# VGLoic/kzg-poly-commit-exploration

Measured on AMD Instinct MI355X. Metric: g1_msm_commitments_per_sec_degree_2^20, higher is better.
Workload: dtype i32 digits (Fp: 13 signed radix-2^30 digits, Montgomery 2^390; Fr: 8 x u32, Montgomery 2^256)

## Files before the change

### kzg_poly_commit_exploration_amd/csrc/api.hip

```cpp
#include <hip/hip_runtime.h>
#include <sys/random.h>

#include <algorithm>
#include <atomic>
#include <cerrno>
#include <chrono>
#include <condition_variable>
#include <cstdio>
#include <cstdlib>
#include <cstring>
#include <deque>
#include <functional>
#include <mutex>
#include <new>
#include <string>
#include <thread>
#include <vector>

#include "../../include/kzg_mi355x.h"
#include "engine.h"
#include "host_field.hpp"
#include "host_fr.hpp"
#include "fr30_host.hpp"
#include "host_pairing.hpp"
// ... 149 lines not shown
    DevBuf lag_part;
    DevBuf gp_in, gp_z, gp_part;
    PinnedBuf gp_flags{PinnedBuf::Mapped};
    DevBuf cpoly, cagg;
    SlotKind kind = SLOT_IDLE;
    size_t job_n = 0;
    uint32_t job_batch = 1;
    uint32_t open_y[8] = {};
    bool timing = false;
    bool has_quotient = false;
    bool tail_checked = false;
    kzg_kernel_times times = {};
};

}

struct kzg_ctx {
    kzg::MultiState* multi = nullptr;
    int device = 0;
    std::mutex mu;
    std::condition_variable slot_cv;
    int sync_owned = 0;
    bool raw_partials = false;
    bool host_trace = false;
    std::atomic<uint64_t> trace_ns[5] = {};
    std::atomic<uint64_t> trace_calls{0};
    std::string last_error;
    size_t n = 0;
    MsmConfig cfg = {};
    DevBuf table;
    DevBuf ntt_tw;
    DevBuf lag_table;
    size_t lag_n = 0;
    uint64_t srs_gen = 0;
    ReducePlan plan;
    size_t arena_records = 0, final_records = 0;
    uint32_t max_batch = 1;
    Slot slots[kNumSlots];
    hipStream_t front_stream = nullptr, heavy_stream = nullptr, tail_stream = nullptr;
    hipStream_t upload_stream = nullptr;
    uint32_t accum_lds_bytes = 41u * 1024u;
    uint32_t small_lds_bytes = 48u * 1024u;
    bool small_msm_off = false;
    bool slots_ready = false;
    bool timing = false;
    std::mutex fk20_mu;
    DevBuf glv;
    uint32_t glv_log = 0;
    DevBuf fk20_B, fk20_tab;
    uint32_t fk20_log_L = 0, fk20_log_l = 0;
    Workspace<11> fk20_ws;
    std::mutex recover_mu;
    DevBuf rec_g;
    Workspace<11> rec_ws;
    Workspace<17> vc_ws;
    Workspace<8> blob_ws;
    std::mutex lookup_mu;
    Workspace<6> lu_ws;
    std::mutex quotient_mu;
    Workspace<11> pq_ws;
    uint32_t pq_zinv_key = ~0u;
};

namespace {

#define HIP_TRY(ctx, expr)                                                                          \
    do {                                                                                            \
        hipError_t _e = (expr);                                                                     \
        if (_e != hipSuccess) {                                                                     \
            (ctx)->last_error = std::string(#expr) + ": " + hipGetErrorString(_e);                  \
            return KZG_ERR_HIP;                                                                     \
        }                                                                                           \
    } while (0)

int hip_fail(kzg_ctx* ctx, const char* what, hipError_t e) {
    ctx->last_error = std::string(what) + ": " + hipGetErrorString(e);
    return KZG_ERR_HIP;
}

struct TmpStream {
    hipStream_t s = nullptr;
    ~TmpStream() { if (s) hipStreamDestroy(s); }
};

int sync_unlocked(kzg_ctx* ctx, std::unique_lock<std::mutex>& lk, hipStream_t st, const char* what) {
    lk.unlock();
    const hipError_t e = hipStreamSynchronize(st);
    lk.lock();
    return e == hipSuccess ? KZG_OK : hip_fail(ctx, what, e);
}
constexpr const char* kCopyCoeffs = "hipMemcpyAsync (coefficients)";
int copy_unlocked(kzg_ctx* ctx, std::unique_lock<std::mutex>& lk, hipStream_t st, void* dst, const void* src, size_t bytes,
                  hipMemcpyKind kind, const char* what) {
    if (!bytes) return KZG_OK;
    lk.unlock();
    const hipError_t e = hipMemcpyAsync(dst, src, bytes, kind, st);
    lk.lock();
    return e == hipSuccess ? KZG_OK : hip_fail(ctx, what, e);
}

void free_slot_msm(Slot& s) {
    for (DevBuf* b : {&s.cnt, &s.offs, &s.block_sums, &s.pairs, &s.sorted, &s.buckets, &s.part_a, &s.part_b, &s.pair_scratch,
                      &s.heavy_ws, &s.arena})
        b->reset();
    s.fin.reset();
}

int create_stream(kzg_ctx* ctx, hipStream_t* out, bool high) {
    int least = 0, greatest = 0;
    HIP_TRY(ctx, hipDeviceGetStreamPriorityRange(&least, &greatest));
    const char* v = std::getenv("KZG_STREAM_PRIORITIES");
    const bool prio = !(v && v[0] == '0');
    HIP_TRY(ctx, hipStreamCreateWithPriority(out, hipStreamNonBlocking, prio ? (high ? greatest : least) : 0));
    return KZG_OK;
}

int ensure_slot_basics(kzg_ctx* ctx, Slot& s) {
    if (s.stream) return KZG_OK;
    if (!ctx->front_stream) {
        int rc = create_stream(ctx, &ctx->front_stream, false);
        if (rc) return rc;
    }
    if (!ctx->upload_stream) HIP_TRY(ctx, hipStreamCreateWithFlags(&ctx->upload_stream, hipStreamNonBlocking));
    for (auto& e : s.ev)
        if (!e) HIP_TRY(ctx, hipEventCreate(&e));
    if (!s.upload_ev) HIP_TRY(ctx, hipEventCreateWithFlags(&s.upload_ev, hipEventDisableTiming));
    s.stream = s.end = ctx->front_stream;
    if (!s.done) HIP_TRY(ctx, hipEventCreateWithFlags(&s.done, hipEventDisableTiming));
    return s.small.reserve(ctx, 64 * 4);
}

int upload_unlocked(kzg_ctx* ctx, std::unique_lock<std::mutex>& lk, Slot& s, void* dst, const void* src, size_t bytes) {
    if (!bytes) return KZG_OK;
    int rc = copy_unlocked(ctx, lk, ctx->upload_stream, dst, src, bytes, hipMemcpyHostToDevice, kCopyCoeffs);
    if (rc) return rc;
    HIP_TRY(ctx, hipEventRecord(s.upload_ev, ctx->upload_stream));
    HIP_TRY(ctx, hipStreamWaitEvent(s.stream, s.upload_ev, 0));
    return KZG_OK;
}

int ensure_poly(kzg_ctx* ctx, Slot& s, size_t n) {
    const size_t cap = n < 1024 ? 1024 : n;
    if (cap * 32 <= s.stage.cap) return KZG_OK;
    if (s.done) HIP_TRY(ctx, hipEventSynchronize(s.done));
    HIP_TRY(ctx, hipStreamSynchronize(ctx->upload_stream));
    HIP_TRY(ctx, hipStreamSynchronize(s.stream));
    for (DevBuf* b : {&s.stage, &s.q, &s.chunk, &s.block}) b->reset();
    int rc = s.stage.reserve(ctx, cap * 32);
    if (rc == KZG_OK) rc = s.q.reserve(ctx, cap * 32);
    if (rc == KZG_OK) rc = s.chunk.reserve(ctx, poly_chunk_words((uint32_t)cap) * 4);
    if (rc == KZG_OK) rc = s.block.reserve(ctx, poly_block_words((uint32_t)cap) * 4);
    if (rc) s.stage.reset();
    return rc;
}

void plan_reduce(kzg_ctx* ctx) {
    ReducePlan P;
    uint32_t bits = 0;
    while ((1u << bits) < ctx->cfg.nb) bits++;
    P.lo_bits = bits / 2;
    P.hi_bits = bits - P.lo_bits;
    P.row_lo = P.hi_bits / 2;
    P.row_hi = P.hi_bits - P.row_lo;
    P.col_lo = P.lo_bits / 2;
    P.col_hi = P.lo_bits - P.col_lo;
    P.off_r2row = 0;
    P.off_c2row = P.off_r2row + (1u << P.row_hi);
    P.off_r2col = P.off_c2row + (1u << P.row_lo);
    P.off_c2col = P.off_r2col + (1u << P.col_hi);
    P.total = P.off_c2col + (1u << P.col_lo);
    ctx->plan = P;
    ctx->arena_records = ((size_t)1 << P.hi_bits) + ((size_t)1 << P.lo_bits);
    ctx->final_records = P.total;
}

int setup_slots_impl(kzg_ctx* ctx);
int setup_slots(kzg_ctx* ctx, bool keep_table_on_failure = false) {
    ctx->slots_ready = false;
    int rc = setup_slots_impl(ctx);
    if (rc != KZG_OK) {
        for (auto& s : ctx->slots) free_slot_msm(s);
        if (keep_table_on_failure) return rc;
        ctx->table.reset();
        ctx->lag_table.reset();
        ctx->lag_n = 0;
        ctx->n = 0;
        (void)hipGetLastError();
    }
    return rc;
}
int setup_slots_impl(kzg_ctx* ctx) {
    plan_reduce(ctx);
    if (const char* v = std::getenv("KZG_TEST_FAIL_SLOT_ALLOC")) {
        const int mode = std::atoi(v);
        if (mode == 1 || (mode == 2 && ctx->max_batch > 1)) {
            ctx->last_error = "injected allocation failure (KZG_TEST_FAIL_SLOT_ALLOC)";
            return KZG_ERR_HIP;
        }
    }
    if (!ctx->heavy_stream) {
        int rc = create_stream(ctx, &ctx->heavy_stream, true);
        if (rc) return rc;
    }
    if (!ctx->tail_stream) {
        int rc = create_stream(ctx, &ctx->tail_stream, false);
        if (rc) return rc;
    }
    const MsmConfig cfg = ctx->cfg;
    if (ctx->max_batch > sort_max_batch(cfg)) ctx->max_batch = sort_max_batch(cfg);
    const size_t B = ctx->max_batch;
    const size_t pairs = (size_t)cfg.max_digits * ctx->n * B;
    for (int i = 0; i < kNumSlots; i++) {
        Slot& s = ctx->slots[i];
        {
            int rcb = ensure_slot_basics(ctx, s);
            if (rcb) return rcb;
        }
        if (!s.sorted_ev) {
            HIP_TRY(ctx, hipEventCreateWithFlags(&s.sorted_ev, hipEventDisableTiming));
            HIP_TRY(ctx, hipEventCreateWithFlags(&s.accum_ev, hipEventDisableTiming));
        }
        free_slot_msm(s);
        int rc = s.cnt.reserve(ctx, (size_t)sort_count_entries((uint32_t)B, cfg) * 4 + 64);
        if (rc == KZG_OK) rc = s.offs.reserve(ctx, ((size_t)cfg.nb * B + 1) * 4);
        if (rc == KZG_OK) rc = s.block_sums.reserve(ctx, (size_t)sort_workspace_words() * 4);
        if (rc) return rc;
        HIP_TRY(ctx, hipMemset(s.block_sums.p, 0, (size_t)sort_workspace_zero_words() * 4));
        rc = s.pairs.reserve(ctx, (pairs ? pairs : 1) * 8);
        if (rc == KZG_OK) rc = s.sorted.reserve(ctx, (pairs ? pairs : 1) * 4);
        if (rc == KZG_OK) rc = s.buckets.reserve(ctx, (size_t)cfg.nb * B * kXyzzBytes);
        if (rc == KZG_OK) rc = s.part_a.reserve(ctx, (size_t)kMaxAccumLanes * kXyzzBytes);
        if (rc == KZG_OK) rc = s.part_b.reserve(ctx, (size_t)kMaxAccumLanes * kXyzzBytes);
        if (rc == KZG_OK) rc = s.pair_scratch.reserve(ctx, accumulate_pair_scratch_bytes(pairs));
        if (rc == KZG_OK) rc = s.heavy_ws.reserve(ctx, heavy_workspace_bytes());
        if (rc == KZG_OK) rc = s.arena.reserve(ctx, ctx->arena_records * B * kXyzzBytes);
        if (rc == KZG_OK) rc = s.fin.reserve(ctx, ctx->final_records * B * kXyzzBytes);
        if (rc) return rc;
        s.kind = SLOT_IDLE;
    }
    ctx->slots_ready = true;
    return KZG_OK;
}

int build_tables(kzg_ctx* ctx, hipStream_t st, void* d_xyzz_tmp, void* d_prefix) {
    const size_t n = ctx->n;
    for (uint32_t j = 1; j < ctx->cfg.W; j++) {
        char* prev = (char*)ctx->table.p + (size_t)(j - 1) * n * kAffineBytes;
        char* next = (char*)ctx->table.p + (size_t)j * n * kAffineBytes;
        launch_table_window(st, prev, (uint32_t)n, ctx->cfg.level_bits, d_xyzz_tmp, d_prefix, next);
    }
    HIP_TRY(ctx, hipGetLastError());
    HIP_TRY(ctx, hipStreamSynchronize(st));
    return KZG_OK;
}

int drain_all(kzg_ctx* ctx) {
    for (hipStream_t st : {ctx->upload_stream, ctx->front_stream, ctx->heavy_stream, ctx->tail_stream})
        if (st) HIP_TRY(ctx, hipStreamSynchronize(st));
    return KZG_OK;
}

static int srs_release(kzg_ctx* ctx) {
    ctx->slots_ready = false;
    int rc = drain_all(ctx);
    if (rc) return rc;
    for (auto& s : ctx->slots) s.kind = SLOT_IDLE;
    ctx->table.reset();
    ctx->fk20_B.reset();
    ctx->fk20_tab.reset();
    ctx->lag_table.reset();
    ctx->lag_n = 0;
    ctx->srs_gen++;
    ctx->n = 0;
    return KZG_OK;
}

int srs_prepare(kzg_ctx* ctx, size_t n) {
    if (n == 0 || n > 0x7fffffffu / 32) return KZG_ERR_INVALID_ARG;
    int rc = srs_release(ctx);
    if (rc) return rc;
    size_t free_b = 0, total_b = 0;
    HIP_TRY(ctx, hipMemGetInfo(&free_b, &total_b));
    size_t budget = (size_t)((double)free_b * 0.6);
    if (const char* v = std::getenv("KZG_TABLE_GB")) budget = (size_t)(std::strtod(v, nullptr) * 1073741824.0);
    MsmConfig cfg = choose_msm_config(n, budget);
    if ((size_t)cfg.W * n >= 0x80000000ull) return KZG_ERR_INVALID_ARG;
    ctx->cfg = cfg;
    return ctx->table.reserve(ctx, (size_t)cfg.W * n * kAffineBytes);
}

struct MsmBasis {
    const void* table;
    uint32_t stride;
};
int enqueue_msm(kzg_ctx* ctx, Slot& s, const uint32_t* d_scalars, int is_mont, size_t n, int ev_base,
                uint32_t batch = 1, uint64_t stride = 0, const MsmBasis* basis = nullptr) {
    const MsmConfig cfg = ctx->cfg;
    const void* table = basis ? basis->table : ctx->table.p;
    const uint32_t table_stride = basis ? basis->stride : (uint32_t)ctx->n;
    const uint32_t nbt = cfg.nb * batch;
    hipStream_t st = s.stream;
    s.end = st;
    if (s.timing) HIP_TRY(ctx, hipEventRecord(s.ev[ev_base], st));
    const bool header_zeroed = launch_bucket_sort(st, d_scalars, is_mont, (uint32_t)n, batch, stride, table_stride, cfg, s.cnt.dev(),
                       s.block_sums.dev(), s.pairs.dev<uint64_t>(), s.offs.dev(), s.sorted.dev(), (uint32_t*)s.heavy_ws.p);
    if (s.timing) {
        HIP_TRY(ctx, hipEventRecord(s.ev[ev_base + 1], st));
        HIP_TRY(ctx, hipEventRecord(s.ev[ev_base + 2], st));
    }
    bool alone = true;
    for (const auto& other : ctx->slots) alone = alone && (&other == &s || other.kind == SLOT_IDLE);
    const uint64_t max_refs = (uint64_t)n * cfg.max_digits * batch;
    const uint32_t lanes = accumulate_lanes(max_refs, alone);
    const ReducePlan& P = ctx->plan;
    const uint32_t R = 1u << P.hi_bits, C = 1u << P.lo_bits, B = batch;
    char* row = (char*)s.arena.p;
    char* col = row + (size_t)R * B * kXyzzBytes;
    char* fin = (char*)s.fin.d;
    const uint32_t rl = 1u << P.row_lo, rh = 1u << P.row_hi, cl = 1u << P.col_lo, ch = 1u << P.col_hi;
    const TreeSumDesc stage1[2] = {
        {s.buckets.p, row, B * R, C, C, 1, B * R, 0},
        {s.buckets.p, col, B * C, R, 1, C, C, (uint64_t)cfg.nb}};
    const TreeSumDesc stage2[4] = {
        {row, fin + (size_t)P.off_r2row * B * kXyzzBytes, B * rh, rl, rl, 1, rh, R},
        {row, fin + (size_t)P.off_c2row * B * kXyzzBytes, B * rl, rh, 1, rl, rl, R},
        {col, fin + (size_t)P.off_r2col * B * kXyzzBytes, B * ch, cl, cl, 1, ch, C},
        {col, fin + (size_t)P.off_c2col * B * kXyzzBytes, B * cl, ch, 1, cl, cl, C}};
    if (!header_zeroed) HIP_TRY(ctx, hipMemsetAsync(s.heavy_ws.p, 0, kHeavyHeaderBytes, st));
    if (max_refs <= kTinyRefs && !ctx->small_msm_off) {
        if (s.timing) HIP_TRY(ctx, hipEventRecord(s.ev[ev_base + 3], st));
        launch_small_msm(st, table, s.sorted.dev(), s.offs.dev(), nbt, lanes, max_refs, s.buckets.p, s.part_a.p, s.part_b.p,
                         s.heavy_ws.p, s.small.dev() + 26, stage1, stage2, ctx->small_lds_bytes);
        if (s.timing) HIP_TRY(ctx, hipEventRecord(s.ev[ev_base + 4], st));
    } else {
        const bool hand_over = !alone;
        hipStream_t hs = hand_over ? ctx->heavy_stream : st;
        if (hand_over) {
            HIP_TRY(ctx, hipEventRecord(s.sorted_ev, st));
            HIP_TRY(ctx, hipStreamWaitEvent(hs, s.sorted_ev, 0));
        }
        if (s.timing) HIP_TRY(ctx, hipEventRecord(s.ev[ev_base + 3], hs));
        launch_bucket_accumulate(hs, table, s.sorted.dev(), s.offs.dev(), nbt, lanes, s.buckets.p, s.part_a.p, s.part_b.p,
                                 ctx->accum_lds_bytes, s.pair_scratch.p, max_refs,
                                 (char*)s.heavy_ws.p + kAccumClockOffset);
        if (s.timing) HIP_TRY(ctx, hipEventRecord(s.ev[ev_base + 4], hs));
        if (hand_over) {
            HIP_TRY(ctx, hipEventRecord(s.accum_ev, hs));
            st = s.end = ctx->tail_stream;
            HIP_TRY(ctx, hipStreamWaitEvent(st, s.accum_ev, 0));
        }
        launch_bucket_finalize(st, s.offs.dev(), nbt, lanes, s.part_a.p, s.part_b.p, s.buckets.p, s.heavy_ws.p, s.small.dev() + 26,
                               finalize_group_size(nbt));
        launch_tree_sums_two_stage(st, stage1, 2, stage2, 4, (uint32_t*)s.heavy_ws.p + 64, alone);
    }
    if (s.timing) HIP_TRY(ctx, hipEventRecord(s.ev[ev_base + 5], st));
    HIP_TRY(ctx, hipGetLastError());
    return KZG_OK;
}

hf::PX host_wsum(const uint64_t* recs, uint32_t len) {
    hf::PX run = hf::px_inf(), acc = hf::px_inf();
    for (uint32_t v = len; v-- > 1;) {
        run = hf::px_add(run, hf::px_from_record(recs + (size_t)v * kXyzzWords64));
        acc = hf::px_add(acc, run);
    }
    return acc;
}
hf::PX host_shift(hf::PX p, uint32_t k) {
    for (uint32_t i = 0; i < k; i++) p = hf::px_double(p);
    return p;
}
hf::P1 finish_msm(const kzg_ctx* ctx, const Slot& s, uint32_t p = 0, uint32_t batch = 1) {
    const ReducePlan& P = ctx->plan;
    const uint64_t* f = s.fin.host<uint64_t>();
    auto at = [&](uint32_t off, uint32_t len) { return f + ((size_t)off * batch + (size_t)p * len) * kXyzzWords64; };
    const uint32_t rh = 1u << P.row_hi, rl = 1u << P.row_lo, ch = 1u << P.col_hi, cl = 1u << P.col_lo;
    hf::PX w_row = hf::px_add(host_shift(host_wsum(at(P.off_r2row, rh), rh), P.row_lo), host_wsum(at(P.off_c2row, rl), rl));
    hf::PX w_col = hf::px_add(host_shift(host_wsum(at(P.off_r2col, ch), ch), P.col_lo), host_wsum(at(P.off_c2col, cl), cl));
    hf::PX total = hf::px_add(host_shift(w_row, P.lo_bits), w_col);
    if (ctx->cfg.recode == kRecodeNaf) total = hf::px_double(total);
    const uint64_t* r2 = at(P.off_r2row, rh);
    for (uint32_t k = 0; k < rh; k++) total = hf::px_add(total, hf::px_from_record(r2 + (size_t)k * kXyzzWords64));
    return ctx->raw_partials ? hf::px_to_jacobian(total) : hf::px_normalize(total);
}

void write_p1(uint64_t out[18], const hf::P1& p) { std::memcpy(out, &p, sizeof p); }

void fill_device_times(Slot& s) {
    s.times.references = s.small.host()[26];
    const uint64_t not_start = (uint64_t)s.small.host()[28] | ((uint64_t)s.small.host()[29] << 32);
    const uint64_t end = (uint64_t)s.small.host()[30] | ((uint64_t)s.small.host()[31] << 32);
    if (not_start != 0 && end > ~not_start) s.times.accumulate_ms = (float)((double)(end - ~not_start) * 1e-5);
}
void fill_accumulate_times(Slot& s) {
    float ms = 0;
    (void)hipEventElapsedTime(&ms, s.ev[3], s.ev[4]);
    s.times.accumulate_events_ms = ms;
    if (s.times.accumulate_ms == 0) s.times.accumulate_ms = ms;
}

void slot_idle(kzg_ctx* ctx, Slot& s) {
    s.kind = SLOT_IDLE;
    ctx->slot_cv.notify_all();
}
int reserve_slot(kzg_ctx* ctx, std::unique_lock<std::mutex>& lk, bool block) {
    for (;;) {
        for (int i = 0; i < kNumSlots; i++)
            if (ctx->slots[i].kind == SLOT_IDLE) {
                ctx->slots[i].kind = SLOT_RESERVED;
                ctx->sync_owned++;
                return i;
            }
        if (!block || ctx->sync_owned == 0) return -1;
        ctx->slot_cv.wait(lk);
    }
}
void release_owned(kzg_ctx* ctx, int slot) {
    if (ctx->slots[slot].kind == SLOT_RESERVED) ctx->slots[slot].kind = SLOT_IDLE;
    ctx->sync_owned--;
    ctx->slot_cv.notify_all();
}
struct SlotLease {
    kzg_ctx* ctx;
    int slot;
    ~SlotLease() { if (slot >= 0) release_owned(ctx, slot); }
};
void quiesce(kzg_ctx* ctx, std::unique_lock<std::mutex>& lk) {
    while (ctx->sync_owned > 0) ctx->slot_cv.wait(lk);
}

bool host_tail_nonzero(const uint64_t* coeffs, size_t from, size_t n) {
    for (size_t i = from; i < n; i++)
        if (coeffs[4 * i] | coeffs[4 * i + 1] | coeffs[4 * i + 2] | coeffs[4 * i + 3]) return true;
    return false;
}

int points_weights(kzg_ctx* ctx, const uint64_t* zs, size_t k, uint64_t* ws ) {
    if (k < 1 || k > KZG_MAX_OPEN_POINTS) {
        ctx->last_error = "multiproof: k must be in [1, KZG_MAX_OPEN_POINTS]";
        return KZG_ERR_INVALID_ARG;
    }
    hf::Fr z[KZG_MAX_OPEN_POINTS], w[KZG_MAX_OPEN_POINTS];
    std::memcpy(z, zs, 32 * k);
    if (!hf::fr_point_weights(z, k, w)) {
        ctx->last_error = "multiproof: two of the points are equal";
        return KZG_ERR_INVALID_ARG;
    }
    std::memcpy(ws, w, 32 * k);
    return KZG_OK;
}
int ensure_points(kzg_ctx* ctx, Slot& s, size_t n, size_t k) {
    int rc = s.roots.reserve(ctx, KZG_MAX_OPEN_POINTS * points_root_bytes());
    if (rc == KZG_OK) rc = s.pvals.reserve(ctx, KZG_MAX_OPEN_POINTS * 32);
    if (rc == KZG_OK) rc = s.pblock.reserve(ctx, k * poly_block_words((uint32_t)(n ? n : 1)) * 4, s.stream);
    return rc;
}
const uint32_t* points_values(const Slot& s, size_t k) { return k == 1 ? s.small.host() + 8 : s.pvals.host(); }
int enqueue_points_scan(kzg_ctx* ctx, Slot& s, const uint32_t* d_coeffs, size_t n, const uint64_t* zs, const uint64_t* ws,
                        size_t k, size_t nq, bool want_q) {
    std::memset(s.small.host(), 0, 64 * 4);
    std::memset(s.pvals.host(), 0, 32 * k);
    if (n == 0) return KZG_OK;
    if (k == 1) {
        uint32_t zw[8];
        std::memcpy(zw, zs, 32);
        uint32_t* q = want_q && n > 1 ? s.q.dev() : nullptr;
        if (!launch_quotient_single(s.stream, d_coeffs, (uint32_t)n, zw, q, s.small.dev())) {
            PolyScratch sc{s.chunk.dev(), s.block.dev(), s.small.dev(), s.small.dev() + 8};
            launch_quotient(s.stream, d_coeffs, (uint32_t)n, zw, q, sc);
        }
    } else {
        points_fill_roots(s.roots.h, zs, ws, (uint32_t)k, (uint32_t)n);
        HIP_TRY(ctx, hipMemcpyAsync(s.roots.d, s.roots.h, k * points_root_bytes(), hipMemcpyHostToDevice, s.stream));
        launch_quotient_points(s.stream, d_coeffs, (uint32_t)n, s.roots.d, (uint32_t)k, want_q ? s.q.dev() : nullptr, (uint32_t)nq,
                               s.pblock.dev(), s.pvals.dev());
    }
    HIP_TRY(ctx, hipGetLastError());
    return KZG_OK;
}

}

__global__ void k_tail_nonzero(const uint32_t* __restrict__ c, uint64_t from, uint64_t n, uint32_t* __restrict__ flag) {
    uint64_t i = from + (uint64_t)blockIdx.x * blockDim.x + threadIdx.x;
    if (i >= n) return;
    const uint4* p = reinterpret_cast<const uint4*>(c) + 2 * i;
    uint4 a = p[0], b = p[1];
    if (a.x | a.y | a.z | a.w | b.x | b.y | b.z | b.w) *flag = 1u;
}

#define KZG_SINGLE_DEVICE_ONLY(ctx)                                                                        \
    do {                                                                                                     \
        if ((ctx) && (ctx)->multi) {                                                                         \
            (ctx)->last_error = "this entry point takes a single-device context (kzg_ctx_create)";           \
            return KZG_ERR_INVALID_ARG;                                                                      \
        }                                                                                                    \
    } while (0)

extern "C" {

const char* kzg_strerror(int status) {
    switch (status) {
        case KZG_OK: return "ok";
        case KZG_ERR_DEGREE_TOO_HIGH:
            return "Setup does not allow for commitment generation of the polynomial. The polynomial degree is too high.";
        case KZG_ERR_CONSTANT_POLY: return "Unable to divide a constant polynomial";
        case KZG_ERR_REMAINDER:
            return "[divide_by_root] Fail to divide the polynomial by a root, constant terms do not add up";
        case KZG_ERR_INVALID_ARG: return "invalid argument";
        case KZG_ERR_NO_DEVICE: return "no HIP device available (this library has no CPU path)";
        case KZG_ERR_HIP: return "HIP runtime error";
        case KZG_ERR_NO_SRS: return "no SRS loaded";
        case KZG_ERR_BUSY: return "slot busy";
        default: return "unknown status";
    }
}

const char* kzg_last_error(const kzg_ctx* ctx) {
    if (!ctx) return "";
    if (ctx->multi && ctx->last_error.empty()) return multi_last_error(ctx->multi);
    return ctx->last_error.c_str();
}

int kzg_ctx_create_multi_ex(const int* devices, int ndev, unsigned flags, kzg_ctx** out) {
    if (!out) return KZG_ERR_INVALID_ARG;
    *out = nullptr;
    if (!devices || ndev <= 0 || (flags & ~(unsigned)KZG_MULTI_REPLICATE_SRS)) return KZG_ERR_INVALID_ARG;
    kzg::MultiState* m = nullptr;
    std::string err;
    int rc = multi_create(devices, ndev, (flags & KZG_MULTI_REPLICATE_SRS) ? kMultiReplicate : kMultiRange, &m, err);
    if (rc != KZG_OK) return rc;
    kzg_ctx* ctx = new kzg_ctx();
    ctx->multi = m;
    ctx->device = devices[0];
    *out = ctx;
    return KZG_OK;
}
int kzg_ctx_create_multi(const int* devices, int ndev, kzg_ctx** out) { return kzg_ctx_create_multi_ex(devices, ndev, 0u, out); }
int kzg_abi_version(void) { return KZG_ABI_VERSION; }
int kzg_num_devices(const kzg_ctx* ctx) { return !ctx ? 0 : (ctx->multi ? multi_num_devices(ctx->multi) : 1); }
uint64_t kzg_rccl_exchanges(const kzg_ctx* ctx) { return (ctx && ctx->multi) ? multi_rccl_exchanges(ctx->multi) : 0; }

int kzg_ctx_create(int device, kzg_ctx** out) {
    if (!out) return KZG_ERR_INVALID_ARG;
    *out = nullptr;
    int count = 0;
    if (hipGetDeviceCount(&count) != hipSuccess || count <= 0) return KZG_ERR_NO_DEVICE;
    if (device < 0 || device >= count) return KZG_ERR_NO_DEVICE;
    if (hipSetDevice(device) != hipSuccess) return KZG_ERR_NO_DEVICE;
    kzg_ctx* ctx = new kzg_ctx();
    ctx->device = device;
    if (const char* v = std::getenv("KZG_ACCUM_LDS_KB")) ctx->accum_lds_bytes = (uint32_t)std::atoi(v) * 1024u;
    if (const char* v = std::getenv("KZG_SMALL_MSM")) ctx->small_msm_off = std::atoi(v) == 0;
    if (const char* v = std::getenv("KZG_HOST_TRACE")) ctx->host_trace = std::atoi(v) != 0;
    if (hipFuncSetAttribute(small_msm_kernel(), hipFuncAttributeMaxDynamicSharedMemorySize, (int)small_msm_lds_bytes()) == hipSuccess)
        ctx->small_lds_bytes = small_msm_lds_bytes();
    else
        (void)hipGetLastError();
    if (!poly_prepare_device() || !points_prepare_device() || !sets_prepare_device()) {
        delete ctx;
        return KZG_ERR_HIP;
    }
    *out = ctx;
    return KZG_OK;
}

void kzg_ctx_destroy(kzg_ctx* ctx) {
    if (!ctx) return;
    if (ctx->multi) {
        multi_destroy(ctx->multi);
        delete ctx;
        return;
    }
    hipSetDevice(ctx->device);
    if (ctx->host_trace && ctx->trace_calls.load()) {
        const double k = 1e-3 / (double)ctx->trace_calls.load();
        std::fprintf(stderr, "[kzg host trace] %llu kzg_commit calls, us per call: wait-for-slot %.1f upload %.1f submit %.1f device %.1f collect %.1f\n",
                     (unsigned long long)ctx->trace_calls.load(), k * ctx->trace_ns[0].load(), k * ctx->trace_ns[1].load(),
                     k * ctx->trace_ns[2].load(), k * ctx->trace_ns[3].load(), k * ctx->trace_ns[4].load());
    }
    for (hipStream_t st : {ctx->upload_stream, ctx->front_stream, ctx->heavy_stream, ctx->tail_stream})
        if (st) hipStreamSynchronize(st);
    for (hipStream_t st : {ctx->upload_stream, ctx->front_stream, ctx->heavy_stream, ctx->tail_stream})
        if (st) hipStreamDestroy(st);
    delete ctx;
}

size_t kzg_srs_len(const kzg_ctx* ctx) { return !ctx ? 0 : (ctx->multi ? multi_srs_len(ctx->multi) : ctx->n); }
int kzg_num_slots(const kzg_ctx*) { return kNumSlots; }

int kzg_msm_config(const kzg_ctx* ctx, int* digit_bits, int* table_levels, size_t* num_buckets, int* recoding) {
    if (ctx && ctx->multi)
        return kzg_msm_config(multi_kid(ctx->multi, 0), digit_bits, table_levels, num_buckets, recoding);
    if (!ctx || !ctx->n) return KZG_ERR_NO_SRS;
    if (digit_bits) *digit_bits = (int)ctx->cfg.c;
    if (table_levels) *table_levels = (int)ctx->cfg.W;
    if (num_buckets) *num_buckets = ctx->cfg.nb;
    if (recoding) *recoding = (int)ctx->cfg.recode;
    return KZG_OK;
}

int kzg_srs_load_g1(kzg_ctx* ctx, const void* first_g1, size_t stride, size_t n) {
    if (!ctx || !first_g1 || stride < 144) return KZG_ERR_INVALID_ARG;
    if (ctx->multi) {
        std::lock_guard<std::mutex> lkm(ctx->mu);
        ctx->last_error.clear();
        return n ? multi_srs_load(ctx->multi, first_g1, stride, n) : KZG_ERR_INVALID_ARG;
    }
    std::unique_lock<std::mutex> lk(ctx->mu);
    quiesce(ctx, lk);
    HIP_TRY(ctx, hipSetDevice(ctx->device));
    int rc = srs_prepare(ctx, n);
    if (rc) return rc;
    std::vector<uint64_t> packed(n * 18);
    for (size_t i = 0; i < n; i++) std::memcpy(&packed[i * 18], (const char*)first_g1 + i * stride, 144);
    DevBuf d_jac, d_prefix, d_xyzz;
    HIP_TRY(ctx, hipMalloc(&d_jac.p, n * 144));
    HIP_TRY(ctx, hipMalloc(&d_prefix.p, n * 64));
    HIP_TRY(ctx, hipMalloc(&d_xyzz.p, n * kXyzzBytes));
    TmpStream st;
    HIP_TRY(ctx, hipStreamCreateWithFlags(&st.s, hipStreamNonBlocking));
    HIP_TRY(ctx, hipMemcpyAsync(d_jac.p, packed.data(), n * 144, hipMemcpyHostToDevice, st.s));
    ctx->n = n;
    launch_jacobian_to_affine(st.s, d_jac.p, (uint32_t)n, ctx->table.p, d_prefix.p);
    rc = build_tables(ctx, st.s, d_xyzz.p, d_prefix.p);
    if (rc) {
        ctx->n = 0;
        return rc;
    }
    return setup_slots(ctx);
}

int kzg_srs_generate_g1(kzg_ctx* ctx, const uint8_t secret_be[32], uint64_t first, size_t n) {
    if (!ctx || !secret_be) return KZG_ERR_INVALID_ARG;
    if (ctx->multi) {
        std::lock_guard<std::mutex> lkm(ctx->mu);
        ctx->last_error.clear();
        return n ? multi_srs_generate(ctx->multi, secret_be, first, n) : KZG_ERR_INVALID_ARG;
    }
    std::unique_lock<std::mutex> lk(ctx->mu);
    quiesce(ctx, lk);
    HIP_TRY(ctx, hipSetDevice(ctx->device));
    int rc = srs_prepare(ctx, n);
    if (rc) return rc;
    uint32_t raw[8];
// ... 6351 lines not shown
```

### kzg_poly_commit_exploration_amd/csrc/engine.h

```cpp
#pragma once
#include <hip/hip_runtime.h>
#include <stddef.h>
#include <stdint.h>

namespace kzg {

constexpr size_t kAffineBytes = 128;
constexpr size_t kAffineU4 = kAffineBytes / 16;
constexpr size_t kXyzzBytes = 256;
constexpr size_t kXyzzU4 = kXyzzBytes / 16;
constexpr size_t kXyzzWords64 = kXyzzBytes / 8;

enum : uint32_t { kRecodeWindows = 0, kRecodeNaf = 1 };
struct MsmConfig {
    uint32_t recode;
    uint32_t c;
    uint32_t W;
    uint32_t level_bits;
    uint32_t nb;
    uint32_t max_digits;
};

MsmConfig choose_msm_config(size_t n_points, size_t table_budget_bytes);

constexpr uint32_t kTinyRefs = 65536;
__host__ __device__ inline uint32_t accumulate_min_seg(uint64_t refs) { return refs <= kTinyRefs ? 4u : 8u; }
__host__ __device__ inline uint32_t accumulate_seg_len(uint32_t M, uint32_t lanes) {
    uint32_t L = (M + lanes - 1) / lanes;
    const uint32_t lo = accumulate_min_seg(M);
    return L < lo ? lo : L;
}

constexpr size_t kHeavyHeaderBytes = 1024;
uint32_t sort_count_entries(uint32_t max_batch, MsmConfig cfg);
uint32_t sort_max_batch(MsmConfig cfg);
uint32_t sort_workspace_words();
uint32_t sort_workspace_zero_words();
bool launch_bucket_sort(hipStream_t s, const uint32_t* d_scalars, int scalars_are_mont, uint32_t n, uint32_t batch,
                        uint64_t stride, uint32_t table_stride, MsmConfig cfg, uint32_t* d_cnt,
                        uint32_t* d_ws, uint64_t* d_pairs, uint32_t* d_offs, uint32_t* d_sorted, uint32_t* d_header);
constexpr uint32_t kMaxAccumLanes = 262144 + 64;
uint32_t accumulate_lanes(uint64_t max_refs, bool alone = false);
size_t accumulate_pair_scratch_bytes(uint64_t max_refs);
void launch_bucket_accumulate(hipStream_t s, const void* d_table, const uint32_t* d_sorted, const uint32_t* d_offs,
                              uint32_t nb, uint32_t lanes, void* d_buckets ,
                              void* d_part_a, void* d_part_b, uint32_t lds_reserve_bytes, void* d_pair_scratch,
                              uint64_t max_refs, void* d_clock = nullptr );
constexpr size_t kAccumClockOffset = 768;
size_t heavy_workspace_bytes();
void launch_bucket_finalize(hipStream_t s, const uint32_t* d_offs, uint32_t nb, uint32_t lanes, const void* d_part_a,
                            const void* d_part_b, void* d_buckets, void* d_heavy_ws,
                            uint32_t* d_refs_out , uint32_t group = 1);
uint32_t finalize_group_size(uint32_t nb);
struct TreeSumDesc;
uint32_t small_msm_lds_bytes();
const void* small_msm_kernel();
void launch_small_msm(hipStream_t s, const void* d_table, const uint32_t* d_sorted, const uint32_t* d_offs, uint32_t nb,
                      uint32_t lanes, uint64_t max_refs, void* d_buckets, void* d_part_a, void* d_part_b, void* d_heavy_ws,
                      uint32_t* d_refs_out, const TreeSumDesc* stage1 , const TreeSumDesc* stage2 ,
                      uint32_t lds_bytes);
struct TreeSumDesc {
    const void* in;
    void* out;
    uint32_t groups, len;
    uint64_t gstride, estride;
    uint32_t inner;
    uint64_t ostride;
};
void launch_tree_sums(hipStream_t s, const TreeSumDesc* descs, uint32_t count, bool dense = false, bool alone = true);
void launch_tree_sums_two_stage(hipStream_t s, const TreeSumDesc* stage1, uint32_t count1, const TreeSumDesc* stage2,
                                uint32_t count2, uint32_t* d_sync, bool alone);

void launch_jacobian_to_affine(hipStream_t s, const void* d_jac, uint32_t n, void* d_affine_out,
                               void* d_prefix_tmp);
void launch_table_window(hipStream_t s, const void* d_prev_affine, uint32_t n, uint32_t c,
                         void* d_xyzz_tmp, void* d_prefix_tmp, void* d_next_affine);
void launch_srs_generate(hipStream_t s, const uint32_t* secret_raw8 , uint64_t first, uint32_t n,
                         void* d_gtable, void* d_xyzz_tmp, void* d_prefix_tmp, void* d_affine_out);
size_t srs_gtable_bytes();
void launch_affine96_to_table(hipStream_t s, const void* d_affine96, uint32_t n, void* d_table);
void launch_uncompress(hipStream_t s, const void* d_compressed, uint32_t n, void* d_table, uint32_t* d_status);

void launch_wire_g1(hipStream_t s, const void* d_in48, const uint32_t* d_src, uint32_t n, void* d_records, uint32_t stride_bytes,
                    uint32_t* d_err);
void launch_wire_fr(hipStream_t s, const void* d_in32, uint32_t n, uint32_t log_row, bool bit_reversed, void* d_out, uint32_t* d_err);

void launch_enc_g1(hipStream_t s, const void* d_affine, uint32_t n, uint32_t log_row, bool bit_reversed, void* d_out48);
void launch_enc_fr(hipStream_t s, const void* d_in, uint32_t n, uint32_t log_row, uint32_t log_cells, bool bit_reversed, void* d_out32,
                   uint32_t* d_err);
struct Fr30;
void launch_poly_trim(hipStream_t s, void* d_coeffs, uint32_t n, uint64_t stride, uint32_t batch, const Fr30* scale, uint32_t* d_out);

void launch_affine_to_p1(hipStream_t s, const void* d_affine, uint32_t n, void* d_p1_out);

struct Fr30;
constexpr uint32_t kNttMaxLog = 22;
constexpr uint32_t kNttTableLen = 2048;
constexpr uint32_t kNttTileLog = 11;
constexpr uint32_t kNttTile = 1u << kNttTileLog;
constexpr uint32_t kNttMaxRadixLog = 9;
struct NttPlan {
    uint32_t passes;
    uint32_t m[3];
};
NttPlan ntt_plan(uint32_t log_n);
bool ntt_prepare_device();
void launch_ntt(hipStream_t s, const uint32_t* d_in, uint32_t* d_out, uint32_t log_n, const void* d_tw, const Fr30& last_c,
                uint32_t* d_buf_a, uint32_t* d_buf_b);

uint32_t cells_chunk_log(uint32_t nq, uint32_t log_l);
uint64_t cells_agg_words(uint32_t nq, uint32_t log_l, uint32_t cells);
void launch_cell_quotients(hipStream_t s, const uint32_t* d_coeffs, uint32_t nq, uint32_t log_n, uint32_t log_l,
                           uint32_t first_cell, uint32_t cells, const void* d_tw, uint32_t* d_agg, uint32_t* d_q,
                           uint64_t stride);
void launch_cells_gather(hipStream_t s, const uint32_t* d_evals, uint32_t* d_out, uint32_t log_n, uint32_t log_l);

struct Glv {
    uint64_t k1[2], k2[2];
};
constexpr uint32_t kFk20CombWindows = 64;
constexpr uint32_t kFk20CombDigits = 8;
constexpr uint32_t kFk20CombEntries = kFk20CombWindows * kFk20CombDigits;
const void* launch_g1_dft(hipStream_t s, const void* d_in, void* d_a, void* d_b, uint32_t log_len, uint64_t batch,
                          const Glv* d_tw, uint32_t log_tw, bool inverse);
void launch_g1_scale(hipStream_t s, void* d_io, uint64_t n, const Glv& k);
void launch_fk20_srs_gather(hipStream_t s, const void* d_table, uint64_t srs_n, uint32_t log_L, uint32_t log_l, void* d_out);
void launch_fk20_comb(hipStream_t s, const void* d_bases, uint32_t log_L, uint32_t log_l, uint64_t first, uint32_t count,
                      void* d_tmp);
const uint32_t* launch_fk20_fr_side(hipStream_t s, const uint32_t* d_coeffs, uint32_t n, uint32_t m, uint32_t log_L,
                                    uint32_t log_l, uint64_t batch, const void* d_tw, const Fr30& inv_L, uint32_t* d_a,
                                    uint32_t* d_b);
void launch_fk20_pointwise(hipStream_t s, const uint32_t* d_scal, const void* d_tab, uint32_t log_L, uint32_t log_l,
                           uint32_t i0, uint32_t ci, uint64_t batch, void* d_part, void* d_out);
void launch_fk20_select(hipStream_t s, const void* d_conv, uint32_t log_L, uint32_t m, uint32_t log_M, uint64_t batch, void* d_H);
void launch_affine_to_xyzz(hipStream_t s, const void* d_affine, uint64_t n, void* d_out);
void launch_xyzz_to_affine(hipStream_t s, const void* d_xyzz, uint32_t n, void* d_out, void* d_prefix);
const uint32_t* launch_fr_dft(hipStream_t s, const uint32_t* d_in, uint32_t* d_a, uint32_t* d_b, uint32_t log_len, uint64_t batch,
                              const void* d_tw);

uint32_t recover_vanish_parts(uint32_t n_missing);
void launch_recover_vanishing(hipStream_t s, const uint32_t* d_missing, uint32_t n_missing, const void* d_tw, uint32_t log_n,
                              uint32_t log_l, const Fr30& gl, uint32_t* d_part, uint32_t* d_z);
void launch_recover_scatter(hipStream_t s, const uint32_t* d_cells, const int32_t* d_pos, const uint32_t* d_zrecv, uint32_t k,
                            uint32_t log_n, uint32_t log_l, uint64_t batch, uint32_t* d_out);
void launch_recover_twist(hipStream_t s, uint32_t* d_io, uint32_t log_n, uint64_t batch, const void* d_gtab, const Fr30& c);
void launch_recover_divide(hipStream_t s, uint32_t* d_io, uint32_t log_n, uint32_t log_l, uint64_t batch, const uint32_t* d_zinv);
void launch_recover_untwist(hipStream_t s, uint32_t* d_io, uint32_t log_n, uint32_t n, uint64_t batch, const void* d_ginv,
                            const Fr30& c, uint32_t* d_coef, bool pad, uint32_t* d_flags);
void launch_recover_gather(hipStream_t s, const uint32_t* d_in, uint32_t* d_out, uint32_t log_n, uint32_t log_l, uint64_t batch);

void launch_vc_ladder(hipStream_t s, const void* d_rec, const uint32_t* d_src, const Glv* d_glv, uint32_t lanes, uint32_t n_check,
                      uint32_t split, void* d_out_a, void* d_out_b, uint32_t* d_err);
void launch_vc_cell_scale(hipStream_t s, const void* d_T, const uint32_t* d_ids, uint32_t D, const Glv* d_tw, uint32_t shift,
                          void* d_out);
void launch_vc_g1_sum(hipStream_t s, const void* d_in, const uint32_t* d_starts, uint32_t groups, void* d_out);
void launch_vc_fr_sum(hipStream_t s, const uint32_t* d_in, const uint32_t* d_order, const Fr30* d_rho, const uint32_t* d_starts,
                      uint32_t groups, uint32_t log_l, uint32_t* d_out);
void launch_vc_fr_twist(hipStream_t s, uint32_t* d_io, const uint32_t* d_ids, uint32_t D, const void* d_itw, uint32_t log_n,
                        uint32_t log_l, const Fr30& inv_l);

void launch_srs_update(hipStream_t s, const uint32_t* tau_raw8, uint64_t first, uint32_t n, const void* d_level0, void* d_out_xyzz);
void launch_srs_check(hipStream_t s, const void* d_level0, uint32_t n, uint32_t* d_err);

constexpr uint32_t kBaryThreads = 256;
constexpr uint32_t kBaryRun = 4;
constexpr uint32_t kBaryTile = kBaryThreads * kBaryRun;
constexpr uint32_t kBaryPartialWords = 12;
inline uint32_t bary_tiles(uint32_t log_n) { return (uint32_t)((((uint64_t)1 << log_n) + kBaryTile - 1) / kBaryTile); }
void launch_bary(hipStream_t s, const uint32_t* d_evals, uint32_t log_n, uint32_t batch, const Fr30* d_zs, const void* d_tw,
                 const Fr30& inv_n, uint32_t* d_partial, uint32_t* d_out);

constexpr uint32_t kLagTile = 1024;
constexpr uint32_t kLagPartialWords = 24;
inline uint32_t lagrange_tiles(uint32_t log_n) { return (uint32_t)((((uint64_t)1 << log_n) + kLagTile - 1) / kLagTile); }
void launch_lagrange_quotient(hipStream_t s, const uint32_t* d_evals, uint32_t log_n, const Fr30& z, const Fr30& y, const Fr30& inv_n,
                              const void* d_tw, uint32_t* d_q, uint32_t* d_partial, uint32_t* d_flags);

constexpr uint32_t kGpTile = 1024;
constexpr uint32_t kGpCarryThreads = 256;
constexpr uint32_t kGpPartialWords = 24;
constexpr uint32_t kGpMaxColumns = 16;
constexpr uint32_t kGpNone = 0xffffffffu;
inline uint32_t gp_tiles(size_t n) { return (uint32_t)((n + kGpTile - 1) / kGpTile); }
struct GpOut {
    uint32_t* d_z;
    uint32_t* d_partial;
    uint32_t* d_flags;
};
void launch_grand_product(hipStream_t s, const uint32_t* d_nums, const uint32_t* d_dens, uint32_t n, uint32_t t, size_t stride,
                          const Fr30& scale, const Fr30& img_one, const GpOut& out);
void launch_permutation_product(hipStream_t s, const uint32_t* d_wires, const uint32_t* d_sigmas, uint32_t log_n, uint32_t t,
                                size_t stride, const Fr30* bk, const Fr30& beta, const Fr30& gamma, const void* d_tw,
                                const Fr30& scale, const Fr30& img_one, const GpOut& out);

constexpr uint32_t kLuTile = 512;
constexpr uint32_t kLuCarryThreads = 256;
constexpr uint32_t kLuMaxColumns = 16;
constexpr uint32_t kLuNone = 0xffffffffu;
constexpr uint32_t kLuRecD = 0, kLuRecHit = 9, kLuRecW = 10, kLuRecC = 20, kLuRecBase = 32, kLuPartialWords = 40;
inline uint32_t lu_tiles(size_t n) { return (uint32_t)((n + kLuTile - 1) / kLuTile); }
struct LuOut {
    uint32_t* d_phi;
    uint32_t* d_partial;
    uint32_t* d_flags;
};
void launch_logderivative_sum(hipStream_t s, const uint32_t* d_nums, const uint32_t* d_dens, uint32_t n, uint32_t t, size_t stride,
                              const Fr30& scale, const Fr30& img_one, const LuOut& out);
void launch_lookup_sum(hipStream_t s, const uint32_t* d_lookups, uint32_t n, uint32_t k, size_t stride, const uint32_t* d_table,
                       const uint32_t* d_mult, const Fr30& beta, const Fr30& scale, const Fr30& img_one, const LuOut& out);
void launch_batch_inverse(hipStream_t s, const uint32_t* d_vals, uint32_t n, const Fr30& scale, const Fr30& img_one, const LuOut& out);
struct LuHash {
    uint32_t* d_slots;
    uint32_t log_cap;
    uint32_t* d_counts;
    uint32_t* d_words;
};
void launch_lookup_multiplicities(hipStream_t s, const uint32_t* d_table, uint32_t n_table, const uint32_t* d_lookups, uint32_t n,
                                  uint32_t k, size_t stride, const LuHash& h, const Fr30& count_img, uint32_t* d_out_mult,
                                  uint32_t* d_out_rows, uint32_t* d_flags);

constexpr uint32_t kPqTile = 256;
constexpr uint32_t kPqMaxColumns = 7;
constexpr uint32_t kPqMaxLogExt = 3;
struct PqColumns {
    const uint32_t *d_wires, *d_sigmas, *d_z, *d_l0, *d_gate, *d_zinv;
};
struct PqScalars {
    const Fr30 *beta, *gamma, *one, *alpha1, *alpha2;
    const Fr30* bkg;
};
void launch_pq_constraints(hipStream_t s, const PqColumns& cols, uint32_t log_N, uint32_t rot, uint32_t t, size_t stride,
                           const PqScalars& sc, const void* d_tw, uint32_t* d_out);
void launch_pq_pad_twist(hipStream_t s, const uint32_t* d_in, size_t stride, uint32_t len, const Fr30& fill, uint32_t log_N,
                         uint64_t batch, const void* d_gtab, const Fr30& c, uint32_t* d_out);

constexpr uint32_t kCombineThreads = 256;
constexpr uint32_t kCombineTile = 2048;
constexpr uint32_t kCombinePartialWords = 12;
constexpr uint32_t kCombineMax = 256;
constexpr uint32_t kCombineTabPa = 0;
constexpr uint32_t kCombineTabPb = 16;
constexpr uint32_t kCombineTabZ256 = 32;
constexpr uint32_t kCombineTabWa = 33;
constexpr uint32_t kCombineTabWb = 49;
constexpr uint32_t kCombineTabW256 = 65;
constexpr uint32_t kCombineTabGamma = 66;
constexpr uint32_t kCombineTabLen = kCombineTabGamma + kCombineMax;
inline uint32_t combine_tiles(uint32_t n) { return (uint32_t)(((uint64_t)n + kCombineTile - 1) / kCombineTile); }
void launch_combine_eval(hipStream_t s, const uint32_t* d_coeffs, uint32_t n, uint32_t t, uint64_t stride, const Fr30* d_tab,
                         uint32_t first, bool carry, uint32_t* d_f, uint32_t* d_partial, uint32_t* d_ys);
constexpr uint32_t kSetsMax = 8;
constexpr uint32_t kSetsMaxPoints = 16;
constexpr uint32_t kSetsMaxValues = kCombineMax * kSetsMaxPoints;
void launch_sets_combine(hipStream_t s, const uint32_t* d_coeffs, uint32_t n, uint32_t t, uint64_t stride, const Fr30* d_tab,
                         const Fr30* d_mult, const uint32_t* d_sel, uint32_t sel_base, bool carry, uint32_t* d_g, uint32_t* d_partial,
                         uint32_t* d_ys);

}
#include <string>
struct kzg_ctx;
namespace kzg {
void ctx_set_raw_partials(kzg_ctx* ctx, bool raw);
int ctx_drop_srs(kzg_ctx* ctx);
int ctx_commit_batch_host(kzg_ctx* ctx, const uint64_t* coeffs, size_t n, size_t stride_coeffs, size_t first, size_t step,
                          size_t count, uint64_t* out_p1s);
int ctx_open_batch_host(kzg_ctx* ctx, const uint64_t* coeffs, size_t n, size_t stride_coeffs, size_t first, size_t step,
                        size_t count, const uint64_t* zs, const uint64_t* ys, uint64_t* out_p1s, int* statuses);
int ctx_open_slice_begin(kzg_ctx* ctx, const uint64_t* slice, size_t len, const uint64_t z[4], uint64_t out_h[4], int* slot_out);
int ctx_open_slice_finish(kzg_ctx* ctx, int slot, size_t len, const uint64_t carry[4], const uint64_t z[4],
                          const uint64_t start[4], uint64_t out_p1[18]);
void ctx_open_slice_abort(kzg_ctx* ctx, int slot);

struct MultiState;
enum : uint32_t { kMultiRange = 0, kMultiReplicate = 1 };
int multi_create(const int* devices, int ndev, uint32_t mode, MultiState** out, std::string& err);
void multi_destroy(MultiState* m);
size_t multi_srs_len(const MultiState* m);
int multi_num_devices(const MultiState* m);
uint64_t multi_rccl_exchanges(const MultiState* m);
kzg_ctx* multi_kid(MultiState* m, int g);
const char* multi_last_error(const MultiState* m);
int multi_srs_generate(MultiState* m, const uint8_t secret_be[32], uint64_t first, size_t n);
int multi_srs_load(MultiState* m, const void* first_g1, size_t stride, size_t n);
int multi_srs_load_affine(MultiState* m, const void* affine_xy, size_t n);
int multi_srs_load_compressed(MultiState* m, const uint8_t* compressed, size_t n, size_t* bad_index);
int multi_srs_read(MultiState* m, size_t index, size_t count, uint64_t* out_p1);
int multi_commit(MultiState* m, const void* scalars, int is_mont, size_t n, uint64_t out_p1[18]);
int multi_open(MultiState* m, const uint64_t* coeffs, size_t n, const uint64_t z[4], const uint64_t y[4], uint64_t out_p1[18]);
int multi_commit_batch(MultiState* m, const uint64_t* coeffs, size_t n, size_t batch, size_t stride_coeffs, uint64_t* out_p1s);
int multi_open_batch(MultiState* m, const uint64_t* coeffs, size_t n, size_t batch, size_t stride_coeffs, const uint64_t* zs,
                     const uint64_t* ys, uint64_t* out_p1s, int* statuses);
int multi_open_points(MultiState* m, const uint64_t* coeffs, size_t n, const uint64_t* zs, const uint64_t* ys, size_t k,
                      uint64_t out_p1[18]);
int multi_open_combined(MultiState* m, const uint64_t* coeffs, size_t n, size_t t, size_t stride, const uint64_t z[4],
                        const uint64_t gamma[4], uint64_t* out_ys, uint64_t out_p1[18]);
int multi_open_sets(MultiState* m, const uint64_t* coeffs, size_t n, size_t t, size_t stride, const uint32_t* set_of,
                    const uint32_t* set_len, size_t nsets, const uint64_t* zs, const uint64_t gamma[4], uint64_t* out_ys,
                    uint64_t out_p1[18]);
int multi_set_max_batch(MultiState* m, size_t max_batch);
uint32_t multi_mode(const MultiState* m);

struct PolyScratch {
    uint32_t* d_chunk;
    uint32_t* d_block;
    uint32_t* d_flags;
    uint32_t* d_result;
};
bool poly_prepare_device();
size_t poly_chunk_words(uint32_t n);
size_t poly_block_words(uint32_t n);
bool launch_quotient_single(hipStream_t s, const uint32_t* d_coeffs, uint32_t n, const uint32_t z_mont[8], uint32_t* d_q,
                            uint32_t* d_small);
void launch_quotient(hipStream_t s, const uint32_t* d_coeffs, uint32_t n, const uint32_t z_mont[8],
                     uint32_t* d_q, PolyScratch scratch);
bool points_prepare_device();
size_t points_root_bytes();
void points_fill_roots(void* h_roots, const uint64_t* zs_mont, const uint64_t* ws_mont, uint32_t k, uint32_t n);
void launch_quotient_points(hipStream_t s, const uint32_t* d_coeffs, uint32_t n, const void* d_roots, uint32_t k, uint32_t* d_q,
                            uint32_t nq, uint32_t* d_block, uint32_t* d_vals);
bool sets_prepare_device();
void launch_quotient_sets(hipStream_t s, const uint32_t* d_g, uint32_t n, const void* d_roots, uint32_t k, uint32_t* d_q,
                          uint32_t* d_block, uint32_t* d_vals);

constexpr uint32_t kBlobProofMaxN = 4096;
constexpr uint32_t kBlobProofZWords = 12;
bool launch_blobproof_quotients(hipStream_t s, const uint32_t* d_coeffs, uint32_t n, uint64_t stride, uint32_t batch,
                                const uint32_t* d_z, uint32_t* d_q, uint32_t* d_flags);

}
```

### kzg_poly_commit_exploration_amd/csrc/msm_accum.hip

```cpp
#include <cstdlib>

#ifndef KZG_ACCUM_PARALLEL_COLUMNS
#define KZG_F30_SERIAL_COLUMNS 1
#endif
#include "engine.h"
#include "field30_inv.hip.h"
#include "g1_30.hip.h"

namespace kzg {

#ifndef KZG_ACCUM_BLOCK
#define KZG_ACCUM_BLOCK 256
#endif
constexpr int kAccumBlock = KZG_ACCUM_BLOCK;

__device__ __forceinline__ Fq load_fq(const uint4* __restrict__ p) {
    const uint4 a = p[0], b = p[1], c = p[2];
    const uint32_t d = reinterpret_cast<const uint32_t*>(p)[12];
    Fq r;
    r.d[0] = (int32_t)a.x; r.d[1] = (int32_t)a.y; r.d[2] = (int32_t)a.z; r.d[3] = (int32_t)a.w;
    r.d[4] = (int32_t)b.x; r.d[5] = (int32_t)b.y; r.d[6] = (int32_t)b.z; r.d[7] = (int32_t)b.w;
    r.d[8] = (int32_t)c.x; r.d[9] = (int32_t)c.y; r.d[10] = (int32_t)c.z; r.d[11] = (int32_t)c.w;
    r.d[12] = (int32_t)d;
    return r;
}
__device__ __forceinline__ Affine30 load_affine30(const uint4* __restrict__ table, uint32_t idx) {
    const uint4* p = table + (size_t)idx * kAffineU4;
    Affine30 r;
    r.x = load_fq(p);
    r.y = load_fq(p + 4);
    return r;
}

__device__ __forceinline__ uint32_t bucket_of(const uint32_t* __restrict__ offs, uint32_t nb, uint32_t pos) {
    uint32_t lo = 0, hi = nb;
    while (hi - lo > 1) {
        uint32_t mid = (lo + hi) >> 1;
        if (offs[mid] <= pos) lo = mid; else hi = mid;
    }
    return lo;
}

typedef __attribute__((address_space(3))) char* lds_char_ptr;
typedef uint32_t accum_u32x4 __attribute__((ext_vector_type(4)));
typedef const __attribute__((address_space(3))) accum_u32x4* lds_u4_ptr;
extern __shared__ uint4 lds_points[];
__device__ __forceinline__ uint32_t accum_wave_lane() { return __builtin_amdgcn_mbcnt_hi(~0u, __builtin_amdgcn_mbcnt_lo(~0u, 0u)); }
__device__ __forceinline__ uint32_t accum_wave_slot() {
    const uint32_t lds0 = (uint32_t)(uintptr_t)(lds_char_ptr)(char*)lds_points;
    return lds0 + __builtin_amdgcn_readfirstlane(threadIdx.x >> 6) * (8u * 64u * 16u);
}
__device__ __forceinline__ void accum_issue_gather(const uint4* __restrict__ table, uint32_t slot, uint32_t r) {
    const char* src = reinterpret_cast<const char*>(table + (size_t)(r & 0x7fffffffu) * kAffineU4);
#pragma unroll
    for (int k = 0; k < 8; k++)
        __builtin_amdgcn_global_load_lds((const __attribute__((address_space(1))) void*)(src + 16 * k),
                                         (__attribute__((address_space(3))) void*)(lds_char_ptr)(uintptr_t)(slot + 1024u * k),
                                         16, 0, 0);
}
constexpr int kFlushOps = 17;
static_assert(kFlushOps == 17, "the literal in accum_take_point's s_waitcnt");
__device__ __forceinline__ Affine30 accum_read_point(uint32_t lane_slot) {
    Affine30 r;
    lds_u4_ptr q = (lds_u4_ptr)(uintptr_t)lane_slot;
    const accum_u32x4 x0 = q[0], x1 = q[64], x2 = q[128], x3 = q[192];
    const accum_u32x4 y0 = q[256], y1 = q[320], y2 = q[384], y3 = q[448];
    r.x.d[0] = (int32_t)x0.x; r.x.d[1] = (int32_t)x0.y; r.x.d[2] = (int32_t)x0.z; r.x.d[3] = (int32_t)x0.w;
    r.x.d[4] = (int32_t)x1.x; r.x.d[5] = (int32_t)x1.y; r.x.d[6] = (int32_t)x1.z; r.x.d[7] = (int32_t)x1.w;
    r.x.d[8] = (int32_t)x2.x; r.x.d[9] = (int32_t)x2.y; r.x.d[10] = (int32_t)x2.z; r.x.d[11] = (int32_t)x2.w;
    r.x.d[12] = (int32_t)x3.x;
    r.y.d[0] = (int32_t)y0.x; r.y.d[1] = (int32_t)y0.y; r.y.d[2] = (int32_t)y0.z; r.y.d[3] = (int32_t)y0.w;
    r.y.d[4] = (int32_t)y1.x; r.y.d[5] = (int32_t)y1.y; r.y.d[6] = (int32_t)y1.z; r.y.d[7] = (int32_t)y1.w;
    r.y.d[8] = (int32_t)y2.x; r.y.d[9] = (int32_t)y2.y; r.y.d[10] = (int32_t)y2.z; r.y.d[11] = (int32_t)y2.w;
    r.y.d[12] = (int32_t)y3.x;
    return r;
}
__device__ __forceinline__ Affine30 accum_take_point(uint32_t slot, bool wave_flushed = false) {
#ifdef KZG_ACCUM_FULL_WAIT
    wave_flushed = false;
#endif
    if (wave_flushed) asm volatile("s_waitcnt vmcnt(17)" ::: "memory");
    else asm volatile("s_waitcnt vmcnt(0)" ::: "memory");
    const Affine30 r = accum_read_point(slot + accum_wave_lane() * 16u);
    asm volatile("s_waitcnt lgkmcnt(0)" ::: "memory");
    return r;
}
struct AccumRare {
    XYZZ30 acc;
    Fq P, Rn;
};
static __device__ __noinline__ bool accum_rare_call(AccumRare* io) { return xyzz30_acc_rare(io->acc, io->P, io->Rn); }
__device__ __forceinline__ void accum_flush_run(uint4* dst, const XYZZ30& a) {
    const Fq* f[4] = {&a.X, &a.Y, &a.ZZ, &a.ZZZ};
    accum_u32x4 v[16];
#pragma unroll
    for (int c = 0; c < 4; c++) {
        v[4 * c + 0] = accum_u32x4{(uint32_t)f[c]->d[0], (uint32_t)f[c]->d[1], (uint32_t)f[c]->d[2], (uint32_t)f[c]->d[3]};
        v[4 * c + 1] = accum_u32x4{(uint32_t)f[c]->d[4], (uint32_t)f[c]->d[5], (uint32_t)f[c]->d[6], (uint32_t)f[c]->d[7]};
        v[4 * c + 2] = accum_u32x4{(uint32_t)f[c]->d[8], (uint32_t)f[c]->d[9], (uint32_t)f[c]->d[10], (uint32_t)f[c]->d[11]};
        v[4 * c + 3] = accum_u32x4{(uint32_t)f[c]->d[12], 0u, 0u, 0u};
    }
    asm volatile(
        "global_store_dwordx4 %0, %1, off\n\t"
        "global_store_dwordx4 %0, %2, off offset:16\n\t"
        "global_store_dwordx4 %0, %3, off offset:32\n\t"
        "global_store_dwordx4 %0, %4, off offset:48\n\t"
        "global_store_dwordx4 %0, %5, off offset:64\n\t"
        "global_store_dwordx4 %0, %6, off offset:80\n\t"
        "global_store_dwordx4 %0, %7, off offset:96\n\t"
        "global_store_dwordx4 %0, %8, off offset:112\n\t"
        "global_store_dwordx4 %0, %9, off offset:128\n\t"
        "global_store_dwordx4 %0, %10, off offset:144\n\t"
        "global_store_dwordx4 %0, %11, off offset:160\n\t"
        "global_store_dwordx4 %0, %12, off offset:176\n\t"
        "global_store_dwordx4 %0, %13, off offset:192\n\t"
        "global_store_dwordx4 %0, %14, off offset:208\n\t"
        "global_store_dwordx4 %0, %15, off offset:224\n\t"
        "global_store_dwordx4 %0, %16, off offset:240"
        :
        : "v"(dst), "v"(v[0]), "v"(v[1]), "v"(v[2]), "v"(v[3]), "v"(v[4]), "v"(v[5]), "v"(v[6]), "v"(v[7]), "v"(v[8]), "v"(v[9]),
          "v"(v[10]), "v"(v[11]), "v"(v[12]), "v"(v[13]), "v"(v[14]), "v"(v[15])
        : "memory");
}
__device__ __forceinline__ uint32_t accum_ref(const uint32_t* __restrict__ sorted, uint32_t i) {
    return *reinterpret_cast<const uint32_t*>(reinterpret_cast<const char*>(sorted) + (uint32_t)(i * 4u));
}

#ifndef KZG_ACCUM_MIN_BLOCKS
#define KZG_ACCUM_MIN_BLOCKS 2
#endif
__global__ void __launch_bounds__(kAccumBlock, KZG_ACCUM_MIN_BLOCKS)
k_bucket_accumulate(const uint4* __restrict__ table, const uint32_t* __restrict__ sorted, const uint32_t* __restrict__ offs,
                    uint32_t nb, uint32_t lanes, uint4* __restrict__ buckets, uint4* __restrict__ part_a,
                    uint4* __restrict__ part_b, unsigned long long* __restrict__ clk) {
    asm volatile("" ::: "v175");
    const bool stamp = clk != nullptr && (threadIdx.x & 63) == 0;
    if (stamp) atomicMax(&clk[0], ~(unsigned long long)wall_clock64());
    const uint32_t lane = blockIdx.x * kAccumBlock + threadIdx.x;
    const uint32_t M = offs[nb];
    const uint32_t L = accumulate_seg_len(M, lanes);
    const uint64_t start64 = (uint64_t)lane * L;
    if (start64 >= M) return;
    const uint32_t start = (uint32_t)start64;
    const uint32_t end = (M - start < L) ? M : start + L;

    uint32_t b = bucket_of(offs, nb, start);
    uint32_t b_beg = offs[b], b_end = offs[b + 1];
    uint32_t b_end_next = offs[(b + 2 <= nb) ? b + 2 : nb];
    uint32_t run_start = start;
    XYZZ30 acc = xyzz30_inf();
    const uint32_t wave_slot = accum_wave_slot();
    uint32_t ref = accum_ref(sorted, start);
    uint32_t ref_next = accum_ref(sorted, min(start + 1, M - 1));
    accum_issue_gather(table, wave_slot, ref);
    for (uint32_t e = start; e < end; e++) {
        const bool wave_flushed = __builtin_amdgcn_ballot_w64(e == b_end) != 0;
        if (e == b_end) {
            uint4* dst = (run_start == b_beg) ? buckets + (size_t)b * kXyzzU4 : part_a + (size_t)lane * kXyzzU4;
            xyzz30_acc_settle(acc);
            accum_flush_run(dst, acc);
            acc = xyzz30_inf();
            b++;
            b_beg = b_end;
            b_end = b_end_next;
            while (b_end <= e) {
                b++;
                b_beg = b_end;
                b_end = offs[b + 1];
            }
            b_end_next = offs[(b + 2 <= nb) ? b + 2 : nb];
            run_start = e;
        }
        Fq P, Rn;
        uint32_t code;
        {
            const Affine30 p = accum_take_point(wave_slot, wave_flushed);
            code = xyzz30_acc_head(acc, p, (ref >> 31) != 0, P, Rn);
        }
        bool more = code == 0;
        if (__builtin_amdgcn_ballot_w64(code != 0) != 0) {
            if (code & kAccFresh) {
                if (!(code & kAccPointInf)) {
                    const Affine30 p = accum_read_point(wave_slot + accum_wave_lane() * 16u);
                    xyzz30_acc_set(acc, p, (ref >> 31) != 0);
                }
            } else if (code == kAccMaybeEqual) {
                AccumRare t;
                t.acc = acc;
                t.P = P;
                t.Rn = Rn;
                more = accum_rare_call(&t);
                acc = t.acc;
                P = t.P;
                Rn = t.Rn;
                __builtin_amdgcn_s_waitcnt(0x0f70);
            }
        }
        ref = ref_next;
        if (e + 1 < end) accum_issue_gather(table, wave_slot, ref);
        ref_next = accum_ref(sorted, min(e + 2, M - 1));
        if (more) xyzz30_acc_tail(acc, P, Rn);
    }
    uint4* dst;
    if (run_start == b_beg && end == b_end) dst = buckets + (size_t)b * kXyzzU4;
    else if (run_start == start) dst = part_a + (size_t)lane * kXyzzU4;
    else dst = part_b + (size_t)lane * kXyzzU4;
    xyzz30_acc_settle(acc);
    store_xyzz30(dst, acc);
    if (stamp) atomicMax(&clk[1], (unsigned long long)wall_clock64());
}

constexpr uint32_t kPairRecU4 = 4;

static __device__ __noinline__ Fq fq_mul_call(Fq a, Fq b) { return fq_mul(a, b); }
static __device__ __noinline__ Fq fq_sqr_call(Fq a) { return fq_sqr(a); }
#ifdef KZG_PAIR_CALLS
#define KZG_PAIR_MUL(a, b) fq_mul_call(a, b)
#define KZG_PAIR_SQR(a) fq_sqr_call(a)
#else
#define KZG_PAIR_MUL(a, b) fq_mul(a, b)
#define KZG_PAIR_SQR(a) fq_sqr(a)
#endif
static __device__ __noinline__ void fq_inv_call(Fq* io) {
    const Fq a = *io;
    *io = fq_inv(a);
}
static __device__ __noinline__ uint32_t pair_classify_call(const Affine30* a, bool nega, const Affine30* b, bool negb, Fq* den) {
    Fq d;
    const uint32_t kind = pair_classify(*a, nega, *b, negb, d);
    *den = d;
    return kind;
}

__global__ void __launch_bounds__(kAccumBlock, 2) k_bucket_accumulate_pairs(const uint4* __restrict__ table,
                                                                            const uint32_t* __restrict__ sorted,
                                                                            const uint32_t* __restrict__ offs, uint32_t nb,
                                                                            uint32_t lanes, uint4* __restrict__ buckets,
                                                                            uint4* __restrict__ part_a,
                                                                            uint4* __restrict__ part_b,
                                                                            uint4* __restrict__ prefix_buf) {
    const uint32_t lane = blockIdx.x * kAccumBlock + threadIdx.x;
    const uint32_t M = offs[nb];
    const uint32_t L = accumulate_seg_len(M, lanes);
    const uint64_t start64 = (uint64_t)lane * L;
    if (start64 >= M) return;
    const uint32_t start = (uint32_t)start64;
    const uint32_t end = (M - start < L) ? M : start + L;
    const uint32_t J = (end - start + 1) / 2;
    auto rec = [&](uint32_t j, uint32_t piece) { return prefix_buf + ((size_t)(j * kPairRecU4 + piece) * lanes + lane); };
    uint4* const slot0 = lds_points + (threadIdx.x >> 6) * (16 * 64);
    uint4* const slot1 = slot0 + 8 * 64;
    const uint32_t wl = threadIdx.x & 63;
    auto dma = [&](uint4* slot, uint32_t r, int first_piece, int pieces) {
        const char* src = reinterpret_cast<const char*>(table + (size_t)(r & 0x7fffffffu) * kAffineU4);
#pragma unroll
        for (int k = 0; k < 8; k++)
            if (k >= first_piece && k < first_piece + pieces)
                __builtin_amdgcn_global_load_lds((const __attribute__((address_space(1))) void*)(src + 16 * k),
                                                 (__attribute__((address_space(3))) void*)(slot + 64 * k), 16, 0, 0);
    };
    auto lds_fq = [&](const uint4* slot, int first_piece) {
        const uint4 a = slot[64 * first_piece + wl], b2 = slot[64 * (first_piece + 1) + wl], c = slot[64 * (first_piece + 2) + wl],
                    d = slot[64 * (first_piece + 3) + wl];
        Fq r;
        r.d[0] = (int32_t)a.x; r.d[1] = (int32_t)a.y; r.d[2] = (int32_t)a.z; r.d[3] = (int32_t)a.w;
        r.d[4] = (int32_t)b2.x; r.d[5] = (int32_t)b2.y; r.d[6] = (int32_t)b2.z; r.d[7] = (int32_t)b2.w;
        r.d[8] = (int32_t)c.x; r.d[9] = (int32_t)c.y; r.d[10] = (int32_t)c.z; r.d[11] = (int32_t)c.w;
        r.d[12] = (int32_t)d.x;
        return r;
    };

    uint32_t b = bucket_of(offs, nb, start);
    uint32_t b_end = offs[b + 1];
    Fq run = fq_one();
    {
        uint32_t r0 = sorted[start], r1 = start + 1 < end ? sorted[start + 1] : 0u;
        uint32_t r0n = start + 2 < end ? sorted[start + 2] : 0u, r1n = start + 3 < end ? sorted[start + 3] : 0u;
        dma(slot0, r0, 0, 4);
        dma(slot1, r1, 0, 4);
        for (uint32_t j = 0; j < J; j++) {
            const uint32_t e0 = start + 2 * j, e1 = e0 + 1;
            while (b_end <= e0) {
                b++;
                b_end = offs[b + 1];
            }
            asm volatile("s_waitcnt vmcnt(0)" ::: "memory");
            const Fq x0 = lds_fq(slot0, 0), x1 = lds_fq(slot1, 0);
            asm volatile("s_waitcnt lgkmcnt(0)" ::: "memory");
            const uint32_t c0 = r0, c1 = r1;
            if (j + 1 < J) {
                r0 = r0n;
                r1 = r1n;
                dma(slot0, r0, 0, 4);
                dma(slot1, r1, 0, 4);
                r0n = e0 + 4 < end ? sorted[e0 + 4] : 0u;
                r1n = e0 + 5 < end ? sorted[e0 + 5] : 0u;
            }
            uint32_t kind = kPairNone;
            Fq den = fq_one();
            if (e1 < end && e1 < b_end) {
                const Fq dx = fq_norm(fq_sub_raw(x1, x0));
                if (!fq_all_zero(x0) && !fq_all_zero(x1) && !fq_is_zero(dx)) {
                    kind = kPairAdd;
                    den = dx;
                } else {
                    Affine30 a, c;
                    a.x = x0;
                    a.y = load_fq(table + (size_t)(c0 & 0x7fffffffu) * kAffineU4 + 4);
                    c.x = x1;
                    c.y = load_fq(table + (size_t)(c1 & 0x7fffffffu) * kAffineU4 + 4);
                    kind = pair_classify_call(&a, (c0 >> 31) != 0, &c, (c1 >> 31) != 0, &den);
                }
            }
            *rec(j, 0) = make_uint4((uint32_t)run.d[0], (uint32_t)run.d[1], (uint32_t)run.d[2], (uint32_t)run.d[3]);
            *rec(j, 1) = make_uint4((uint32_t)run.d[4], (uint32_t)run.d[5], (uint32_t)run.d[6], (uint32_t)run.d[7]);
            *rec(j, 2) = make_uint4((uint32_t)run.d[8], (uint32_t)run.d[9], (uint32_t)run.d[10], (uint32_t)run.d[11]);
            *rec(j, 3) = make_uint4((uint32_t)run.d[12], kind, c0, c1);
            if (kind == kPairAdd || kind == kPairDouble) run = KZG_PAIR_MUL(run, den);
        }
    }
    Fq inv = run;
    fq_inv_call(&inv);

    b = bucket_of(offs, nb, end - 1);
    uint32_t b_beg = offs[b];
    b_end = offs[b + 1];
    XYZZ30 acc = xyzz30_inf();
    auto flush = [&]() {
        uint4* dst;
        if (b_beg >= start && b_end <= end) dst = buckets + (size_t)b * kXyzzU4;
        else if (b_beg <= start) dst = part_a + (size_t)lane * kXyzzU4;
        else dst = part_b + (size_t)lane * kXyzzU4;
        store_xyzz30(dst, acc);
    };
    auto enter = [&](uint32_t e) {
        if (e < b_beg) {
            flush();
            acc = xyzz30_inf();
            do {
                b--;
                b_end = b_beg;
                b_beg = offs[b];
            } while (b_beg > e);
        }
    };
    uint32_t e = end - 1;
    auto ref_at = [&](uint32_t idx_plus_1) { return idx_plus_1 > start ? sorted[idx_plus_1 - 1] : 0u; };
    uint32_t w0 = sorted[e], w1 = ref_at(e), w2 = e >= 1 ? ref_at(e - 1) : 0u, w3 = e >= 2 ? ref_at(e - 2) : 0u;
    uint4 q0, q1, q2, q3;
    {
        const uint32_t j = (e - start) >> 1;
        q0 = *rec(j, 0); q1 = *rec(j, 1); q2 = *rec(j, 2); q3 = *rec(j, 3);
        dma(slot1, w0, 0, 8);
        dma(slot0, w1, 0, 8);
    }
    bool more_steps = true;
    while (more_steps) {
        asm volatile("s_waitcnt vmcnt(0)" ::: "memory");
        const uint32_t j = (e - start) >> 1;
        const uint32_t kind = q3.y;
        const bool second = ((e - start) & 1u) != 0;
        const bool paired = kind != kPairNone && second;
        const uint32_t r_hi = w0, r_lo = w1;
        Fq prefix;
        prefix.d[0] = (int32_t)q0.x; prefix.d[1] = (int32_t)q0.y; prefix.d[2] = (int32_t)q0.z; prefix.d[3] = (int32_t)q0.w;
        prefix.d[4] = (int32_t)q1.x; prefix.d[5] = (int32_t)q1.y; prefix.d[6] = (int32_t)q1.z; prefix.d[7] = (int32_t)q1.w;
        prefix.d[8] = (int32_t)q2.x; prefix.d[9] = (int32_t)q2.y; prefix.d[10] = (int32_t)q2.z; prefix.d[11] = (int32_t)q2.w;
        prefix.d[12] = (int32_t)q3.x;
        Affine30 pt;
        pt.x = lds_fq(slot1, 0);
        pt.y = lds_fq(slot1, 4);
        Affine30 lo;
        lo.x = lds_fq(slot0, 0);
        lo.y = lds_fq(slot0, 4);
        asm volatile("s_waitcnt lgkmcnt(0)" ::: "memory");
        enter(e);
        const uint32_t used = paired ? 2u : 1u;
        more_steps = e >= start + used;
        if (more_steps) {
            e -= used;
            if (paired) { w0 = w2; w1 = w3; } else { w0 = w1; w1 = w2; w2 = w3; }
            const uint32_t jn = (e - start) >> 1;
            q0 = *rec(jn, 0); q1 = *rec(jn, 1); q2 = *rec(jn, 2); q3 = *rec(jn, 3);
            dma(slot1, w0, 0, 8);
            dma(slot0, w1, 0, 8);
            if (paired) {
                w2 = e >= start + 2 ? sorted[e - 2] : 0u;
                w3 = e >= start + 3 ? sorted[e - 3] : 0u;
            } else {
                w3 = e >= start + 3 ? sorted[e - 3] : 0u;
            }
        }
        bool neg = (r_hi >> 31) != 0;
        bool have = true;
        if (paired) {
            const bool n0 = (r_lo >> 31) != 0;
            if (kind == kPairCancel) {
                have = false;
            } else if (kind == kPairOnlyA) {
                pt = lo;
                neg = n0;
            } else if (kind != kPairOnlyB) {
                const Fq den = kind == kPairAdd ? fq_norm(fq_sub_raw(pt.x, lo.x)) : fq_norm(fq_add_raw(fq_cneg(lo.y, n0), fq_cneg(pt.y, neg)));
                const Fq inv_den = KZG_PAIR_MUL(inv, prefix);
                KZG_SB30();
                inv = KZG_PAIR_MUL(inv, den);
                KZG_SB30();
                pt = pair_sum_with(kind, lo, n0, pt, neg, inv_den, [](const Fq& x, const Fq& y) { return KZG_PAIR_MUL(x, y); },
                                   [](const Fq& x) { return KZG_PAIR_SQR(x); });
                neg = false;
            }
        }
        if (have) xyzz30_madd(acc, pt, neg);
    }
    flush();
}

__global__ void __launch_bounds__(64) k_fq_table_to_p1(const uint4* __restrict__ table, uint32_t n, uint4* __restrict__ out) {
    const uint32_t i = blockIdx.x * 64 + threadIdx.x;
    if (i >= n) return;
    const Affine30 a = load_affine30(table, i);
    uint32_t w[36];
#pragma unroll
    for (int t = 0; t < 36; t++) w[t] = 0;
    if (!(fq_all_zero(a.x) && fq_all_zero(a.y))) {
        fq_to_u32x12(a.x, w);
        fq_to_u32x12(a.y, w + 12);
        constexpr uint32_t ONE[12] = {0x0002fffdu, 0x76090000u, 0xc40c0002u, 0xebf4000bu, 0x53c758bau, 0x5f489857u,
                                      0x70525745u, 0x77ce5853u, 0xa256ec6du, 0x5c071a97u, 0xfa80e493u, 0x15f65ec3u};
#pragma unroll
        for (int t = 0; t < 12; t++) w[24 + t] = ONE[t];
    }
    uint4* o = out + (size_t)i * 9;
#pragma unroll
    for (int t = 0; t < 9; t++) o[t] = make_uint4(w[4 * t], w[4 * t + 1], w[4 * t + 2], w[4 * t + 3]);
}
void launch_affine_to_p1(hipStream_t s, const void* d_affine, uint32_t n, void* d_p1) {
    if (!n) return;
    hipLaunchKernelGGL(k_fq_table_to_p1, dim3((n + 63) / 64), dim3(64), 0, s, (const uint4*)d_affine, n, (uint4*)d_p1);
}

uint32_t accumulate_lanes(uint64_t max_refs, bool alone) {
    (void)alone;
    static const uint64_t target = [] {
        const char* v = std::getenv("KZG_ACCUM_LANES");
        uint64_t l = v ? std::strtoull(v, nullptr, 10) : 131072ull;
        return l < 64 ? 131072ull : (l > 262144ull ? 262144ull : l);
    }();
    const uint64_t lo = accumulate_min_seg(max_refs);
    uint64_t lanes = (max_refs + lo - 1) / lo;
    if (lanes > target) lanes = target;
    lanes = (lanes + kAccumBlock - 1) / kAccumBlock * kAccumBlock;
    return (uint32_t)lanes;
}

bool accumulate_pairs_enabled() {
    static const int pairs_mode = [] {
        const char* v = std::getenv("KZG_ACCUM_PAIRS");
        return v ? std::atoi(v) : 0;
    }();
    return pairs_mode != 0;
}
size_t accumulate_pair_scratch_bytes(uint64_t max_refs) {
    if (!accumulate_pairs_enabled()) return 0;
    return (size_t)(max_refs / 2 + kMaxAccumLanes) * kPairRecU4 * 16;
}

void launch_bucket_accumulate(hipStream_t s, const void* d_table, const uint32_t* d_sorted, const uint32_t* d_offs,
                              uint32_t nb, uint32_t lanes, void* d_buckets, void* d_part_a, void* d_part_b,
                              uint32_t lds_reserve_bytes, void* d_pair_scratch, uint64_t max_refs, void* d_clock) {
    if (!lanes) return;
    if (accumulate_pairs_enabled() && d_pair_scratch && max_refs / lanes >= 16) {
        hipLaunchKernelGGL(k_bucket_accumulate_pairs, dim3(lanes / kAccumBlock), dim3(kAccumBlock),
                           (kAccumBlock / 64) * 16 * 64 * 16 , s,
                           reinterpret_cast<const uint4*>(d_table), d_sorted, d_offs, nb, lanes,
                           reinterpret_cast<uint4*>(d_buckets), reinterpret_cast<uint4*>(d_part_a),
                           reinterpret_cast<uint4*>(d_part_b), reinterpret_cast<uint4*>(d_pair_scratch));
        return;
    }
    const uint32_t need = (kAccumBlock / 64) * 8 * 64 * 16;
    lds_reserve_bytes = lds_reserve_bytes / (256 / kAccumBlock);
    if (lds_reserve_bytes < need) lds_reserve_bytes = need;
    hipLaunchKernelGGL(k_bucket_accumulate, dim3(lanes / kAccumBlock), dim3(kAccumBlock), lds_reserve_bytes, s,
                       reinterpret_cast<const uint4*>(d_table), d_sorted, d_offs, nb, lanes,
                       reinterpret_cast<uint4*>(d_buckets), reinterpret_cast<uint4*>(d_part_a),
                       reinterpret_cast<uint4*>(d_part_b), reinterpret_cast<unsigned long long*>(d_clock));
}

}
```

### kzg_poly_commit_exploration_amd/csrc/msm_sort.hip

```cpp
#include <cstdlib>
#include <cstring>

#include "engine.h"
#include "fr30.hip.h"

namespace kzg {

typedef uint32_t u32;
#ifndef KZG_DEV
#define KZG_DEV __device__ __forceinline__
#endif

static uint32_t ilog2(uint32_t v) {
    uint32_t b = 0;
    while ((1u << b) < v) b++;
    return b;
}

MsmConfig choose_msm_config(size_t n, size_t table_budget_bytes) {
    const char* force_mode = std::getenv("KZG_MSM_RECODE");
    const char* force_c = std::getenv("KZG_MSM_C");
    const uint32_t fc = force_c ? (uint32_t)std::strtoul(force_c, nullptr, 10) : 0u;
    const bool naf = force_mode && !std::strcmp(force_mode, "naf") && n * 255ull < 0x80000000ull &&
                     (double)n * 255.0 * (double)kAffineBytes <= (double)table_budget_bytes;
    uint32_t best_c = 8;
    const uint32_t best_mode = naf ? kRecodeNaf : kRecodeWindows;
    double best = 1e300;
    for (uint32_t c = 8; c <= (naf ? 21u : 20u); c++) {
        if (fc >= 8 && fc <= (naf ? 21u : 20u) && c != fc) continue;
        if (!naf && !fc && 254u - c * ((255 + c - 1) / c - 1) < 4u) continue;
        double cost = naf ? (double)n * (255.0 / (c + 1) + 0.5) + 8.0 * (double)(1u << (c - 2))
                          : (double)n * ((255 + c - 1) / c) + 20.0 * (double)(1u << (c - 1));
        if (cost < best) {
            best = cost;
            best_c = c;
        }
    }
    MsmConfig cfg;
    cfg.recode = best_mode;
    cfg.c = best_c;
    if (best_mode == kRecodeNaf) {
        cfg.W = 255;
        cfg.level_bits = 1;
        cfg.nb = 1u << (best_c - 2);
        cfg.max_digits = (255 + best_c - 1) / best_c + 1;
    } else {
        cfg.W = (255 + best_c - 1) / best_c;
        cfg.level_bits = best_c;
        cfg.nb = 1u << (best_c - 1);
        cfg.max_digits = cfg.W;
    }
    return cfg;
}

KZG_DEV bool load_scalar(const uint32_t* d_scalars, uint64_t i, int is_mont, u32 k[8]) {
    const uint4* p = reinterpret_cast<const uint4*>(d_scalars) + 2 * (size_t)i;
    const uint4 lo = p[0], hi = p[1];
    const uint32_t in[8] = {lo.x, lo.y, lo.z, lo.w, hi.x, hi.y, hi.z, hi.w};
    const Fr30 d = fr30_from_limbs_raw(in);
    const Fr30 v = is_mont ? fr30_mul(d, fr30_small(1 << 14)) : fr30_mul(d, fr30_const_one270());
    return fr30_abs_to_limbs(v, k);
}

template <class F>
KZG_DEV void for_each_window_digit(u32 k[8], uint32_t c, uint32_t W, F&& f) {
    const u32 mask = (1u << c) - 1u;
    const u32 half = 1u << (c - 1);
    u32 carry = 0;
    for (uint32_t j = 0; j < W; j++) {
        u32 v = (k[0] & mask) + carry;
#pragma unroll
        for (int t = 0; t < 7; t++) k[t] = (k[t] >> c) | (k[t + 1] << (32 - c));
        k[7] >>= c;
        bool neg = v > half;
        u32 mag = neg ? (mask + 1u - v) : v;
        carry = neg ? 1u : 0u;
        if (mag) f(j, mag - 1u, neg);
    }
}

template <class F>
KZG_DEV void for_each_naf_digit(const u32 k[8], uint32_t c, F&& f) {
    const u32 mask = (1u << c) - 1u;
    const u32 half = 1u << (c - 1);
    u32 carry = 0;
    uint32_t p = 0;
#pragma unroll
    for (int t = 0; t < 8; t++) {
        const uint64_t win = ((uint64_t)(t < 7 ? k[t + 1] : 0u) << 32) | k[t];
        while (p < 32) {
            u32 x = (u32)(win >> p);
            if (carry) x = ~x;
            uint32_t z = x ? (uint32_t)__builtin_ctz(x) : 32u;
            if (z >= 32u - p) {
                p = 32;
                break;
            }
            p += z;
            u32 v = ((u32)(win >> p) & mask) + carry;
            const bool neg = v > half;
            const u32 mag = neg ? (mask + 1u - v) : v;
            carry = neg ? 1u : 0u;
            f(32u * (uint32_t)t + p, (mag - 1u) >> 1, neg);
            p += c;
        }
        p -= 32;
    }
}

template <class F>
KZG_DEV void for_each_digit(u32 k[8], MsmConfig cfg, F&& f) {
    if (cfg.recode == kRecodeNaf) for_each_naf_digit(k, cfg.c, f);
    else for_each_window_digit(k, cfg.c, cfg.W, f);
}

constexpr int kSortBlock = 256;
constexpr int kRecodeBlock = 1024;
#ifndef KZG_SORT_TILES
#define KZG_SORT_TILES 512
#endif
constexpr uint32_t kMaxTiles = KZG_SORT_TILES;
constexpr int kMaxCoarse = 2048;
constexpr int kFineMax = 256;

struct SortGeom {
    uint32_t tile;
    uint32_t tiles;
    uint32_t fine_bits;
    uint32_t coarse_bins;
    bool packed;
};

constexpr uint32_t kPackedFineBits = 7, kPackedIndexBits = 24;
static uint32_t sort_fine_bits(MsmConfig cfg, bool packed) {
    const uint32_t bits = ilog2(cfg.nb), most = packed ? kPackedFineBits : 8u;
    return bits < most ? bits : most;
}
static bool sort_packed_buckets(uint32_t nb_total, MsmConfig cfg);

static bool sort_packed_buckets(uint32_t nb_total, MsmConfig cfg) { return (nb_total >> sort_fine_bits(cfg, true)) <= (uint32_t)kMaxCoarse; }

static SortGeom sort_geometry(uint64_t total, uint32_t nb_total, MsmConfig cfg, uint32_t table_stride) {
    SortGeom g;
    static const bool allow_packed = [] { const char* v = std::getenv("KZG_SORT_PACKED"); return !(v && v[0] == '0'); }();
    g.packed = allow_packed && sort_packed_buckets(nb_total, cfg) && (uint64_t)cfg.W * table_stride <= (1ull << kPackedIndexBits);
    uint32_t tile = (uint32_t)((total + kMaxTiles - 1) / kMaxTiles);
    tile = ((tile + kSortBlock - 1) / kSortBlock) * kSortBlock;
    if (tile < (uint32_t)kSortBlock) tile = kSortBlock;
    g.tile = tile;
    g.tiles = (uint32_t)((total + tile - 1) / tile);
    g.fine_bits = sort_fine_bits(cfg, g.packed);
    g.coarse_bins = nb_total >> g.fine_bits;
    return g;
}

uint32_t sort_max_batch(MsmConfig cfg) {
    uint32_t fine_bits = sort_fine_bits(cfg, false);
    uint32_t b = (uint32_t)kMaxCoarse / (cfg.nb >> fine_bits);
    return b < 1 ? 1 : b;
}

uint32_t sort_count_entries(uint32_t max_batch, MsmConfig cfg) {
    uint32_t bins = 0;
    for (uint32_t b = 1; b <= max_batch; b++) {
        const uint32_t nbt = cfg.nb * b;
        const uint32_t q = nbt >> sort_fine_bits(cfg, sort_packed_buckets(nbt, cfg));
        if (q > bins) bins = q;
    }
    return bins * (kMaxTiles + 1u);
}

struct BatchGeom {
    uint32_t n;
    uint32_t batch;
    uint64_t stride;
    uint32_t nb;
};

__global__ void __launch_bounds__(kRecodeBlock) k_sort_count(const uint32_t* __restrict__ d_scalars, int is_mont,
                                                           BatchGeom bg, MsmConfig cfg, uint32_t tile,
                                                           uint32_t fine_bits, uint32_t coarse_bins,
                                                           uint32_t* __restrict__ d_cnt, uint32_t* __restrict__ d_binfill ,
                                                           uint32_t* __restrict__ d_header) {
    __shared__ u32 s_hist[kMaxCoarse];
    if (blockIdx.x == 0 && threadIdx.x < kHeavyHeaderBytes / 4) d_header[threadIdx.x] = 0;
    for (uint32_t q = threadIdx.x; q < coarse_bins; q += kRecodeBlock) s_hist[q] = 0;
    __syncthreads();
    const uint64_t base = (uint64_t)blockIdx.x * tile;
    const uint64_t total = (uint64_t)bg.n * bg.batch;
    for (uint32_t off = threadIdx.x; off < tile; off += kRecodeBlock) {
        uint64_t g = base + off;
        if (g >= total) break;
        uint32_t p = (uint32_t)(g / bg.n);
        uint32_t i = (uint32_t)(g - (uint64_t)p * bg.n);
        u32 k[8];
        (void)load_scalar(d_scalars, p * bg.stride + i, is_mont, k);
        const u32 pb = p * bg.nb;
        for_each_digit(k, cfg, [&](uint32_t, u32 bkt, bool) { atomicAdd(&s_hist[(pb + bkt) >> fine_bits], 1u); });
    }
    __syncthreads();
    for (uint32_t q = threadIdx.x; q < coarse_bins; q += kRecodeBlock) {
        const u32 c = s_hist[q];
        d_cnt[(size_t)blockIdx.x * coarse_bins + q] = c ? atomicAdd(&d_binfill[q], c) : 0u;
    }
}

template <int N>
__device__ __forceinline__ u32 block_exclusive_scan_n(u32 v, u32* lds, u32& total);
__device__ __forceinline__ u32 block_exclusive_scan_256(u32 v, u32* lds, u32& total);

constexpr uint32_t kFineMaxChunks = 4096;
constexpr uint32_t kFineLocal = 16;
constexpr uint32_t kWsBinStart = 0;
constexpr uint32_t kWsPrefix = kMaxCoarse + 8;
constexpr uint32_t kWsBinFill = 2 * kMaxCoarse + 32;
constexpr uint32_t kWsTable = 3 * kMaxCoarse + 64;
uint32_t sort_workspace_words() { return kWsTable + kFineMaxChunks * (uint32_t)kFineMax + 64; }
uint32_t sort_workspace_zero_words() { return kWsTable; }

template <int BLOCK>
KZG_DEV void spread_tile_cursors(uint32_t coarse_bins, const uint32_t* __restrict__ d_cnt, const uint32_t* __restrict__ d_binfill,
                                 uint32_t ch, uint32_t* __restrict__ d_binstart, uint32_t* __restrict__ d_prefix,
                                 uint32_t* __restrict__ d_total, u32* s_cur , u32* s_scan ) {
    const uint32_t t = threadIdx.x;
    constexpr uint32_t kStripes = kMaxCoarse / BLOCK;
    u32 below[kStripes], all[kStripes];
#pragma unroll
    for (uint32_t s = 0; s < kStripes; s++) {
        const uint32_t q = t + s * BLOCK;
        all[s] = q < coarse_bins ? d_binfill[q] : 0u;
        below[s] = q < coarse_bins ? d_cnt[(size_t)blockIdx.x * coarse_bins + q] : 0u;
    }
    u32 carry = 0, chunk_carry = 0;
#pragma unroll
    for (uint32_t s = 0; s < kStripes; s++) {
        if (s * BLOCK >= coarse_bins) break;
        const uint32_t q = t + s * BLOCK;
        u32 stripe_total;
        const u32 start = carry + block_exclusive_scan_n<BLOCK>(all[s], s_scan, stripe_total);
        __syncthreads();
        if (q < coarse_bins) s_cur[q] = start + below[s];
        if (blockIdx.x == 0) {
            const u32 nch = q < coarse_bins ? (all[s] + ch - 1) / ch : 0u;
            u32 chunk_total;
            const u32 cstart = chunk_carry + block_exclusive_scan_n<BLOCK>(nch, s_scan, chunk_total);
            __syncthreads();
            if (q < coarse_bins) {
                d_binstart[q] = start;
                d_prefix[q] = cstart;
            }
            chunk_carry += chunk_total;
        }
        carry += stripe_total;
    }
    if (blockIdx.x == 0 && t == 0) {
        d_binstart[coarse_bins] = carry;
        d_prefix[coarse_bins] = chunk_carry;
        *d_total = carry;
    }
    __syncthreads();
}

__global__ void __launch_bounds__(kRecodeBlock) k_sort_spread(const uint32_t* __restrict__ d_scalars, int is_mont,
                                                            BatchGeom bg, uint32_t table_stride, MsmConfig cfg,
                                                            uint32_t tile, uint32_t tiles, uint32_t fine_bits,
                                                            uint32_t coarse_bins, const uint32_t* __restrict__ d_cnt ,
                                                            const uint32_t* __restrict__ d_binfill ,
                                                            uint32_t ch, uint32_t* __restrict__ d_binstart,
                                                            uint32_t* __restrict__ d_prefix, uint32_t* __restrict__ d_total,
                                                            uint64_t* __restrict__ d_pairs, int packed) {
    __shared__ u32 s_cur[kMaxCoarse];
    __shared__ u32 s_scan[kRecodeBlock];
    spread_tile_cursors<kRecodeBlock>(coarse_bins, d_cnt, d_binfill, ch, d_binstart, d_prefix, d_total, s_cur, s_scan);
    const uint64_t base = (uint64_t)blockIdx.x * tile;
    const uint64_t total = (uint64_t)bg.n * bg.batch;
    const u32 fine_mask = (1u << fine_bits) - 1u;
    for (uint32_t off = threadIdx.x; off < tile; off += kRecodeBlock) {
        uint64_t g = base + off;
        if (g >= total) break;
        uint32_t p = (uint32_t)(g / bg.n);
        uint32_t i = (uint32_t)(g - (uint64_t)p * bg.n);
        u32 k[8];
        const bool flip = load_scalar(d_scalars, p * bg.stride + i, is_mont, k);
        const u32 pb = p * bg.nb;
        for_each_digit(k, cfg, [&](uint32_t j, u32 bkt, bool neg) {
            u32 b = pb + bkt;
            u32 pos = atomicAdd(&s_cur[b >> fine_bits], 1u);
            u32 ref = (j * table_stride + i) | ((neg != flip) ? 0x80000000u : 0u);
            if (packed) reinterpret_cast<u32*>(d_pairs)[pos] = ref | ((b & fine_mask) << kPackedIndexBits);
            else d_pairs[pos] = ((uint64_t)(b & fine_mask) << 32) | ref;
        });
    }
}

constexpr int kStageBlock = 512;
constexpr uint32_t kStageSlots = 7680;

template <int BLOCK>
KZG_DEV u32 block_exclusive_scan_fast(u32 v, u32* s_wave , u32& total) {
    const uint32_t t = threadIdx.x, lane = t & 63u, w = t >> 6;
    u32 incl = v;
#pragma unroll
    for (uint32_t off = 1; off < 64; off <<= 1) {
        const u32 up = __shfl_up(incl, off, 64);
        if (lane >= off) incl += up;
    }
    if (lane == 63) s_wave[w] = incl;
    __syncthreads();
    u32 base = 0, all = 0;
#pragma unroll
    for (uint32_t i = 0; i < BLOCK / 64; i++) {
        const u32 x = s_wave[i];
        if (i < w) base += x;
        all += x;
    }
    __syncthreads();
    total = all;
    return base + incl - v;
}

__global__ void __launch_bounds__(kStageBlock) k_sort_spread_staged(const uint32_t* __restrict__ d_scalars, int is_mont,
                                                                  BatchGeom bg, uint32_t table_stride, MsmConfig cfg,
                                                                  uint32_t tile, uint32_t fine_bits, uint32_t coarse_bins,
                                                                  const uint32_t* __restrict__ d_cnt, const uint32_t* __restrict__ d_binfill,
                                                                  uint32_t ch, uint32_t* __restrict__ d_binstart,
                                                                  uint32_t* __restrict__ d_prefix, uint32_t* __restrict__ d_total,
                                                                  uint32_t* __restrict__ d_pairs32) {
    __shared__ u32 s_cur[kMaxCoarse];
    __shared__ u32 s_cnt[kMaxCoarse];
    __shared__ u32 s_gd[kMaxCoarse];
    __shared__ u32 s_scan[kStageBlock];
    __shared__ u32 s_stage[kStageSlots];
    __shared__ uint16_t s_sbin[kStageSlots];
    spread_tile_cursors<kStageBlock>(coarse_bins, d_cnt, d_binfill, ch, d_binstart, d_prefix, d_total, s_cur, s_scan);
    const uint32_t t = threadIdx.x;
    const uint64_t base = (uint64_t)blockIdx.x * tile;
    const uint64_t total = (uint64_t)bg.n * bg.batch;
    const u32 fine_mask = (1u << fine_bits) - 1u;
    const uint32_t per_round = kStageSlots / cfg.max_digits < (uint32_t)kStageBlock ? kStageSlots / cfg.max_digits : (uint32_t)kStageBlock;
    constexpr uint32_t kBinsPerLane = kMaxCoarse / kStageBlock;
    for (uint32_t r0 = 0; r0 < tile; r0 += per_round) {
        for (uint32_t q = t; q < coarse_bins; q += kStageBlock) s_cnt[q] = 0;
        __syncthreads();
        const uint32_t off = r0 + t;
        const uint64_t g = base + off;
        const bool valid = t < per_round && off < tile && g < total;
        u32 k[8];
        bool flip = false;
        uint32_t i = 0;
        u32 pb = 0;
        if (valid) {
            const uint32_t p = (uint32_t)(g / bg.n);
            i = (uint32_t)(g - (uint64_t)p * bg.n);
            pb = p * bg.nb;
            flip = load_scalar(d_scalars, p * bg.stride + i, is_mont, k);
            u32 k1[8];
#pragma unroll
            for (int w = 0; w < 8; w++) k1[w] = k[w];
            for_each_digit(k1, cfg, [&](uint32_t, u32 bkt, bool) { atomicAdd(&s_cnt[(pb + bkt) >> fine_bits], 1u); });
        }
        __syncthreads();
        u32 mine[kBinsPerLane], sum = 0;
#pragma unroll
        for (uint32_t e = 0; e < kBinsPerLane; e++) {
            const uint32_t q = t * kBinsPerLane + e;
            mine[e] = q < coarse_bins ? s_cnt[q] : 0u;
            sum += mine[e];
        }
        u32 round_total;
        u32 run = block_exclusive_scan_fast<kStageBlock>(sum, s_scan, round_total);
#pragma unroll
        for (uint32_t e = 0; e < kBinsPerLane; e++) {
            const uint32_t q = t * kBinsPerLane + e;
            if (q < coarse_bins) {
                const u32 cur = s_cur[q];
                s_gd[q] = cur - run;
                s_cur[q] = cur + mine[e];
                s_cnt[q] = run;
            }
            run += mine[e];
        }
        __syncthreads();
        if (valid) {
            for_each_digit(k, cfg, [&](uint32_t j, u32 bkt, bool neg) {
                const u32 b = pb + bkt, bin = b >> fine_bits;
                const u32 slot = atomicAdd(&s_cnt[bin], 1u);
                s_stage[slot] = (j * table_stride + i) | ((neg != flip) ? 0x80000000u : 0u) | ((b & fine_mask) << kPackedIndexBits);
                s_sbin[slot] = (uint16_t)bin;
            });
        }
        __syncthreads();
        for (uint32_t e = t; e < round_total; e += kStageBlock) d_pairs32[s_gd[s_sbin[e]] + e] = s_stage[e];
    }
}


static uint32_t fine_chunk_len(uint64_t max_pairs) {
    static const uint64_t target = [] {
        const char* v = std::getenv("KZG_FINE_CHUNKS");
        uint64_t t = v ? std::strtoull(v, nullptr, 10) : 2048ull;
        return t < 1 ? 1ull : (t > 2048 ? 2048ull : t);
    }();
    uint64_t ch = (max_pairs + target - 1) / target;
    ch = (ch + 255) / 256 * 256;
    return (uint32_t)(ch < 4096 ? 4096 : ch);
}

struct FineChunk {
    uint32_t bin, beg, end, nch, j, base;
};
KZG_DEV bool locate_chunk(uint32_t k, const uint32_t* __restrict__ d_prefix, const uint32_t* __restrict__ d_binstart,
                          uint32_t coarse_bins, uint32_t ch, FineChunk& c) {
    if (k >= d_prefix[coarse_bins]) return false;
    uint32_t lo = 0, hi = coarse_bins;
    while (hi - lo > 1) {
        uint32_t mid = (lo + hi) >> 1;
        if (d_prefix[mid] <= k) lo = mid; else hi = mid;
    }
    c.bin = lo;
    c.base = d_prefix[lo];
    c.nch = d_prefix[lo + 1] - c.base;
    c.j = k - c.base;
    const uint32_t rs = d_binstart[lo], re = d_binstart[lo + 1];
    c.beg = rs + c.j * ch;
    c.end = (re - c.beg < ch) ? re : c.beg + ch;
    return true;
}

template <bool kPacked> struct SortPair;
template <> struct SortPair<false> {
    typedef uint64_t type;
    static KZG_DEV u32 key(uint64_t p) { return (u32)(p >> 32); }
    static KZG_DEV u32 ref(uint64_t p) { return (u32)p; }
};
template <> struct SortPair<true> {
    typedef uint32_t type;
    static KZG_DEV u32 key(uint32_t p) { return (p >> kPackedIndexBits) & ((1u << kPackedFineBits) - 1u); }
    static KZG_DEV u32 ref(uint32_t p) { return p & (0x80000000u | ((1u << kPackedIndexBits) - 1u)); }
};

template <bool kPacked>
__global__ void __launch_bounds__(kSortBlock) k_fine_count(const typename SortPair<kPacked>::type* __restrict__ d_pairs,
                                                           const uint32_t* __restrict__ d_binstart, uint32_t fine_bits,
                                                           uint32_t coarse_bins, uint32_t ch,
                                                           const uint32_t* __restrict__ d_prefix,
                                                           uint32_t* __restrict__ d_table, uint32_t* __restrict__ d_binfill) {
    __shared__ u32 s_hist[kFineMax];
    if (blockIdx.x == 0)
        for (uint32_t q = threadIdx.x; q < coarse_bins; q += kSortBlock) d_binfill[q] = 0;
    FineChunk c;
    if (!locate_chunk(blockIdx.x, d_prefix, d_binstart, coarse_bins, ch, c)) return;
    const uint32_t fine = 1u << fine_bits;
    if (threadIdx.x < fine) s_hist[threadIdx.x] = 0;
    __syncthreads();
    for (uint32_t e = c.beg + threadIdx.x; e < c.end; e += kSortBlock) atomicAdd(&s_hist[SortPair<kPacked>::key(d_pairs[e])], 1u);
    __syncthreads();
    if (threadIdx.x < fine) d_table[(size_t)c.base * fine + (size_t)threadIdx.x * c.nch + c.j] = s_hist[threadIdx.x];
}

__global__ void __launch_bounds__(kSortBlock) k_fine_binscan(const uint32_t* __restrict__ d_binstart, uint32_t fine_bits,
                                                             const uint32_t* __restrict__ d_prefix,
                                                             uint32_t* __restrict__ d_table, uint32_t* __restrict__ d_offs) {
    __shared__ u32 s_scan[kSortBlock];
    const uint32_t bin = blockIdx.x, t = threadIdx.x;
    const uint32_t fine = 1u << fine_bits;
    const uint32_t base = d_prefix[bin], nch = d_prefix[bin + 1] - base;
    const uint32_t rs = d_binstart[bin];
    if (nch == 0) {
        if (t < fine) d_offs[bin * fine + t] = rs;
        return;
    }
    if (nch <= kFineLocal) return;
    u32* h = d_table + (size_t)base * fine;
    const uint32_t len = fine * nch;
    const uint32_t per = (len + kSortBlock - 1) / kSortBlock;
    const uint32_t lo = t * per < len ? t * per : len, hi = lo + per < len ? lo + per : len;
    u32 sum = 0;
    for (uint32_t i = lo; i < hi; i++) sum += h[i];
    u32 total;
    u32 run = rs + block_exclusive_scan_256(sum, s_scan, total);
    for (uint32_t i = lo; i < hi; i++) {
        const u32 v = h[i];
        h[i] = run;
        run += v;
    }
}

constexpr uint32_t kFineStage = 4096;
template <bool kPacked>
__global__ void __launch_bounds__(kSortBlock) k_fine_scatter(const typename SortPair<kPacked>::type* __restrict__ d_pairs,
                                                             const uint32_t* __restrict__ d_binstart,
                                                             uint32_t fine_bits, uint32_t coarse_bins, uint32_t ch,
                                                             const uint32_t* __restrict__ d_prefix,
                                                             const uint32_t* __restrict__ d_table,
                                                             uint32_t* __restrict__ d_offs,
                                                             uint32_t* __restrict__ d_sorted) {
    __shared__ u32 s_cur[kFineMax];
    __shared__ u32 s_cnt[kFineMax];
    __shared__ u32 s_ref[kFineStage];
    __shared__ u32 s_dst[kFineStage];
    FineChunk c;
    if (!locate_chunk(blockIdx.x, d_prefix, d_binstart, coarse_bins, ch, c)) return;
    const uint32_t fine = 1u << fine_bits;
    const uint32_t t = threadIdx.x;
    {
        u32 mine = 0;
        if (c.nch <= kFineLocal) {
            u32 row = 0, front = 0;
            if (t < fine) {
                const u32* h = d_table + (size_t)c.base * fine + (size_t)t * c.nch;
                for (uint32_t i = 0; i < c.nch; i++) {
                    const u32 v = h[i];
                    row += v;
                    if (i < c.j) front += v;
                }
            }
            u32 total;
            const u32 key_start = d_binstart[c.bin] + block_exclusive_scan_256(row, s_ref, total);
            __syncthreads();
            mine = key_start + front;
            if (c.j == 0 && t < fine) d_offs[c.bin * fine + t] = key_start;
        } else if (t < fine) {
            mine = d_table[(size_t)c.base * fine + (size_t)t * c.nch + c.j];
            if (c.j == 0) d_offs[c.bin * fine + t] = mine;
        }
        if (t < fine) s_cur[t] = mine;
    }
    for (uint32_t r0 = c.beg; r0 < c.end; r0 += kFineStage) {
        const uint32_t r1 = (c.end - r0 < kFineStage) ? c.end : r0 + kFineStage;
        if (t < kFineMax) s_cnt[t] = 0;
        __syncthreads();
        typename SortPair<kPacked>::type pr[kFineStage / kSortBlock];
#pragma unroll
        for (uint32_t q = 0; q < kFineStage / kSortBlock; q++) {
            const uint32_t e = r0 + q * kSortBlock + t;
            pr[q] = e < r1 ? d_pairs[e] : (typename SortPair<kPacked>::type)0;
            if (e < r1) atomicAdd(&s_cnt[SortPair<kPacked>::key(pr[q])], 1u);
        }
        __syncthreads();
        u32 mine = t < kFineMax ? s_cnt[t] : 0u;
        u32 incl = mine;
        __syncthreads();
        if (t < kFineMax) s_ref[t] = incl;
        __syncthreads();
        for (uint32_t off = 1; off < kFineMax; off <<= 1) {
            u32 add = (t < kFineMax && t >= off) ? s_ref[t - off] : 0u;
            __syncthreads();
            if (t < kFineMax) {
                incl += add;
                s_ref[t] = incl;
            }
            __syncthreads();
        }
        const u32 excl = incl - mine;
        u32 gbase = 0;
        if (t < kFineMax) {
            gbase = s_cur[t];
            s_cur[t] = gbase + mine;
            s_cnt[t] = excl;
        }
        __syncthreads();
        if (t < kFineMax) s_dst[t] = gbase - excl;
        __syncthreads();
        u32 keep_dst[kFineStage / kSortBlock];
        u32 keep_pos[kFineStage / kSortBlock];
#pragma unroll
        for (uint32_t q = 0; q < kFineStage / kSortBlock; q++) {
            const uint32_t e = r0 + q * kSortBlock + t;
            if (e < r1) {
                const u32 key = SortPair<kPacked>::key(pr[q]);
                const u32 pos = atomicAdd(&s_cnt[key], 1u);
                keep_pos[q] = pos;
                keep_dst[q] = s_dst[key] + pos;
            }
        }
        __syncthreads();
#pragma unroll
        for (uint32_t q = 0; q < kFineStage / kSortBlock; q++) {
            const uint32_t e = r0 + q * kSortBlock + t;
            if (e < r1) {
                s_ref[keep_pos[q]] = SortPair<kPacked>::ref(pr[q]);
                s_dst[keep_pos[q]] = keep_dst[q];
            }
        }
        __syncthreads();
        const uint32_t cnt = r1 - r0;
        for (uint32_t i = t; i < cnt; i += kSortBlock) d_sorted[s_dst[i]] = s_ref[i];
        __syncthreads();
    }
}

template <int N>
__device__ __forceinline__ u32 block_exclusive_scan_n(u32 v, u32* lds, u32& total) {
    int t = threadIdx.x;
    lds[t] = v;
    __syncthreads();
    for (int off = 1; off < N; off <<= 1) {
        u32 add = t >= off ? lds[t - off] : 0u;
        __syncthreads();
        lds[t] += add;
        __syncthreads();
    }
    total = lds[N - 1];
    return lds[t] - v;
}
__device__ __forceinline__ u32 block_exclusive_scan_256(u32 v, u32* lds, u32& total) { return block_exclusive_scan_n<256>(v, lds, total); }

constexpr uint32_t kSmallSortScalars = 4096;
constexpr uint32_t kSmallSortBuckets = 4096;
constexpr int kSmallSortBlock = 1024;

__global__ void __launch_bounds__(kSmallSortBlock) k_sort_small(const uint32_t* __restrict__ d_scalars, int is_mont, uint32_t n,
                                                                uint32_t table_stride, MsmConfig cfg,
                                                                uint32_t* __restrict__ d_offs,
                                                                uint32_t* __restrict__ d_sorted,
                                                                uint32_t* __restrict__ d_header) {
    __shared__ u32 s_hist[kSmallSortBuckets];
    if (blockIdx.x == 0 && threadIdx.x < kHeavyHeaderBytes / 4) d_header[threadIdx.x] = 0;
    __shared__ u32 s_part[kSmallSortBlock];
    const uint32_t t = threadIdx.x;
    const uint32_t nb = cfg.nb;
    for (uint32_t b = t; b < nb; b += kSmallSortBlock) s_hist[b] = 0;
    __syncthreads();
    for (uint32_t i = t; i < n; i += kSmallSortBlock) {
        u32 k[8];
        (void)load_scalar(d_scalars, i, is_mont, k);
        for_each_digit(k, cfg, [&](uint32_t, u32 bkt, bool) { atomicAdd(&s_hist[bkt], 1u); });
    }
    __syncthreads();
    const uint32_t per = (nb + kSmallSortBlock - 1) / kSmallSortBlock;
    u32 local = 0;
    for (uint32_t q = 0; q < per; q++) {
        uint32_t b = t * per + q;
        if (b < nb) local += s_hist[b];
    }
    s_part[t] = local;
    __syncthreads();
    for (int off = 1; off < kSmallSortBlock; off <<= 1) {
        u32 add = t >= (uint32_t)off ? s_part[t - off] : 0u;
        __syncthreads();
        s_part[t] += add;
        __syncthreads();
    }
    u32 run = s_part[t] - local;
    for (uint32_t q = 0; q < per; q++) {
        uint32_t b = t * per + q;
        if (b < nb) {
            u32 c = s_hist[b];
            d_offs[b] = run;
            s_hist[b] = run;
            run += c;
        }
    }
    if (t == kSmallSortBlock - 1) d_offs[nb] = s_part[t];
    __syncthreads();
    const uint32_t b_lo = (uint32_t)((uint64_t)nb * blockIdx.x / gridDim.x), b_hi = (uint32_t)((uint64_t)nb * (blockIdx.x + 1) / gridDim.x);
    for (uint32_t i = t; i < n; i += kSmallSortBlock) {
        u32 k[8];
        const bool flip = load_scalar(d_scalars, i, is_mont, k);
        for_each_digit(k, cfg, [&](uint32_t j, u32 bkt, bool neg) {
            if (bkt >= b_lo && bkt < b_hi) {
                u32 pos = atomicAdd(&s_hist[bkt], 1u);
                d_sorted[pos] = (j * table_stride + i) | ((neg != flip) ? 0x80000000u : 0u);
            }
        });
    }
}

bool launch_bucket_sort(hipStream_t s, const uint32_t* d_scalars, int is_mont, uint32_t n, uint32_t batch,
                        uint64_t stride, uint32_t table_stride, MsmConfig cfg, uint32_t* d_cnt, uint32_t* d_ws,
                        uint64_t* d_pairs, uint32_t* d_offs, uint32_t* d_sorted, uint32_t* d_header) {
    if (n == 0 || batch == 0) return false;
    static const bool small_path = [] { const char* v = std::getenv("KZG_SMALL_SORT"); return !(v && v[0] == '0'); }();
    if (small_path && batch == 1 && n <= kSmallSortScalars && cfg.nb <= kSmallSortBuckets) {
        uint32_t groups = n / 256;
        groups = groups < 1 ? 1 : (groups > 8 ? 8 : groups);
        hipLaunchKernelGGL(k_sort_small, dim3(groups), dim3(kSmallSortBlock), 0, s, d_scalars, is_mont, n, table_stride, cfg, d_offs,
                           d_sorted, d_header);
        return true;
    }
    const uint32_t nb_total = cfg.nb * batch;
    SortGeom g = sort_geometry((uint64_t)n * batch, nb_total, cfg, table_stride);
    BatchGeom bg{n, batch, stride, cfg.nb};
    uint32_t* d_binstart = d_ws + kWsBinStart;
    uint32_t* d_prefix = d_ws + kWsPrefix;
    uint32_t* d_table = d_ws + kWsTable;
    uint32_t* d_total = d_offs + nb_total;
    const uint64_t max_pairs = (uint64_t)n * batch * cfg.max_digits;
    const uint32_t ch = fine_chunk_len(max_pairs);
    const uint32_t max_chunks = (uint32_t)((max_pairs + ch - 1) / ch) + g.coarse_bins;
    uint32_t* d_binfill = d_ws + kWsBinFill;
    hipLaunchKernelGGL(k_sort_count, dim3(g.tiles), dim3(kRecodeBlock), 0, s, d_scalars, is_mont, bg, cfg, g.tile,
                       g.fine_bits, g.coarse_bins, d_cnt, d_binfill, d_header);
    static const bool staged = [] { const char* v = std::getenv("KZG_SPREAD_STAGED"); return !(v && v[0] == '0'); }();
    if (g.packed && staged && cfg.max_digits <= kStageSlots)
        hipLaunchKernelGGL(k_sort_spread_staged, dim3(g.tiles), dim3(kStageBlock), 0, s, d_scalars, is_mont, bg, table_stride, cfg,
                           g.tile, g.fine_bits, g.coarse_bins, d_cnt, d_binfill, ch, d_binstart, d_prefix, d_total,
                           reinterpret_cast<uint32_t*>(d_pairs));
    else
        hipLaunchKernelGGL(k_sort_spread, dim3(g.tiles), dim3(kRecodeBlock), 0, s, d_scalars, is_mont, bg, table_stride, cfg,
                           g.tile, g.tiles, g.fine_bits, g.coarse_bins, d_cnt, d_binfill, ch, d_binstart, d_prefix, d_total, d_pairs,
                           g.packed ? 1 : 0);
    if (g.packed)
        hipLaunchKernelGGL(k_fine_count<true>, dim3(max_chunks), dim3(kSortBlock), 0, s, reinterpret_cast<const uint32_t*>(d_pairs),
                           d_binstart, g.fine_bits, g.coarse_bins, ch, d_prefix, d_table, d_binfill);
    else
        hipLaunchKernelGGL(k_fine_count<false>, dim3(max_chunks), dim3(kSortBlock), 0, s, d_pairs, d_binstart, g.fine_bits,
                           g.coarse_bins, ch, d_prefix, d_table, d_binfill);
    hipLaunchKernelGGL(k_fine_binscan, dim3(g.coarse_bins), dim3(kSortBlock), 0, s, d_binstart, g.fine_bits, d_prefix, d_table, d_offs);
    if (g.packed)
        hipLaunchKernelGGL(k_fine_scatter<true>, dim3(max_chunks), dim3(kSortBlock), 0, s, reinterpret_cast<const uint32_t*>(d_pairs),
                           d_binstart, g.fine_bits, g.coarse_bins, ch, d_prefix, d_table, d_offs, d_sorted);
    else
        hipLaunchKernelGGL(k_fine_scatter<false>, dim3(max_chunks), dim3(kSortBlock), 0, s, d_pairs, d_binstart, g.fine_bits,
                           g.coarse_bins, ch, d_prefix, d_table, d_offs, d_sorted);
    return true;
}

}
```

Baseline: 427.7.

## Precompute per-lane start buckets during sort and add single-block fine-bin path

Sort kernels now write, for each accumulate lane, the bucket containing that lane's first reference, so the accumulate kernels no longer binary-search the offsets array at startup. The pairs kernel replaces its second binary search with a forward walk. A new k_fine_bin kernel sorts small coarse bins entirely in one block, so the chunked count/scan/scatter path only handles oversized bins. This trades extra sort-side work and workspace for less accumulate prologue latency and fewer chunked passes.

New measurement: 433.6 (median of 6 runs). No clear change (+1.4%).

```diff
diff --git a/kzg_poly_commit_exploration_amd/csrc/api.hip b/kzg_poly_commit_exploration_amd/csrc/api.hip
--- a/kzg_poly_commit_exploration_amd/csrc/api.hip
+++ b/kzg_poly_commit_exploration_amd/csrc/api.hip
@@ -475,16 +475,16 @@
     hipStream_t st = s.stream;
     s.end = st;
     if (s.timing) HIP_TRY(ctx, hipEventRecord(s.ev[ev_base], st));
-    const bool header_zeroed = launch_bucket_sort(st, d_scalars, is_mont, (uint32_t)n, batch, stride, table_stride, cfg, s.cnt.dev(),
-                       s.block_sums.dev(), s.pairs.dev<uint64_t>(), s.offs.dev(), s.sorted.dev(), (uint32_t*)s.heavy_ws.p);
-    if (s.timing) {
-        HIP_TRY(ctx, hipEventRecord(s.ev[ev_base + 1], st));
-        HIP_TRY(ctx, hipEventRecord(s.ev[ev_base + 2], st));
-    }
     bool alone = true;
     for (const auto& other : ctx->slots) alone = alone && (&other == &s || other.kind == SLOT_IDLE);
     const uint64_t max_refs = (uint64_t)n * cfg.max_digits * batch;
     const uint32_t lanes = accumulate_lanes(max_refs, alone);
+    const bool header_zeroed = launch_bucket_sort(st, d_scalars, is_mont, (uint32_t)n, batch, stride, table_stride, cfg, s.cnt.dev(),
+                       s.block_sums.dev(), s.pairs.dev<uint64_t>(), s.offs.dev(), s.sorted.dev(), (uint32_t*)s.heavy_ws.p, lanes);
+    if (s.timing) {
+        HIP_TRY(ctx, hipEventRecord(s.ev[ev_base + 1], st));
+        HIP_TRY(ctx, hipEventRecord(s.ev[ev_base + 2], st));
+    }
     const ReducePlan& P = ctx->plan;
     const uint32_t R = 1u << P.hi_bits, C = 1u << P.lo_bits, B = batch;
     char* row = (char*)s.arena.p;
@@ -513,7 +513,7 @@
             HIP_TRY(ctx, hipStreamWaitEvent(hs, s.sorted_ev, 0));
         }
         if (s.timing) HIP_TRY(ctx, hipEventRecord(s.ev[ev_base + 3], hs));
-        launch_bucket_accumulate(hs, table, s.sorted.dev(), s.offs.dev(), nbt, lanes, s.buckets.p, s.part_a.p, s.part_b.p,
+        launch_bucket_accumulate(hs, table, s.sorted.dev(), s.offs.dev(), s.block_sums.dev() + sort_seg_bucket_offset(), nbt, lanes, s.buckets.p, s.part_a.p, s.part_b.p,
                                  ctx->accum_lds_bytes, s.pair_scratch.p, max_refs,
                                  (char*)s.heavy_ws.p + kAccumClockOffset);
         if (s.timing) HIP_TRY(ctx, hipEventRecord(s.ev[ev_base + 4], hs));
diff --git a/kzg_poly_commit_exploration_amd/csrc/engine.h b/kzg_poly_commit_exploration_amd/csrc/engine.h
--- a/kzg_poly_commit_exploration_amd/csrc/engine.h
+++ b/kzg_poly_commit_exploration_amd/csrc/engine.h
@@ -35,15 +35,17 @@
 uint32_t sort_count_entries(uint32_t max_batch, MsmConfig cfg);
 uint32_t sort_max_batch(MsmConfig cfg);
 uint32_t sort_workspace_words();
+uint32_t sort_seg_bucket_offset();
 uint32_t sort_workspace_zero_words();
 bool launch_bucket_sort(hipStream_t s, const uint32_t* d_scalars, int scalars_are_mont, uint32_t n, uint32_t batch,
                         uint64_t stride, uint32_t table_stride, MsmConfig cfg, uint32_t* d_cnt,
-                        uint32_t* d_ws, uint64_t* d_pairs, uint32_t* d_offs, uint32_t* d_sorted, uint32_t* d_header);
+                        uint32_t* d_ws, uint64_t* d_pairs, uint32_t* d_offs, uint32_t* d_sorted, uint32_t* d_header,
+                        uint32_t lanes);
 constexpr uint32_t kMaxAccumLanes = 262144 + 64;
 uint32_t accumulate_lanes(uint64_t max_refs, bool alone = false);
 size_t accumulate_pair_scratch_bytes(uint64_t max_refs);
 void launch_bucket_accumulate(hipStream_t s, const void* d_table, const uint32_t* d_sorted, const uint32_t* d_offs,
-                              uint32_t nb, uint32_t lanes, void* d_buckets ,
+                              const uint32_t* d_seg_bucket , uint32_t nb, uint32_t lanes, void* d_buckets ,
                               void* d_part_a, void* d_part_b, uint32_t lds_reserve_bytes, void* d_pair_scratch,
                               uint64_t max_refs, void* d_clock = nullptr );
 constexpr size_t kAccumClockOffset = 768;
diff --git a/kzg_poly_commit_exploration_amd/csrc/msm_accum.hip b/kzg_poly_commit_exploration_amd/csrc/msm_accum.hip
--- a/kzg_poly_commit_exploration_amd/csrc/msm_accum.hip
+++ b/kzg_poly_commit_exploration_amd/csrc/msm_accum.hip
@@ -32,13 +32,9 @@
     return r;
 }
 
-__device__ __forceinline__ uint32_t bucket_of(const uint32_t* __restrict__ offs, uint32_t nb, uint32_t pos) {
-    uint32_t lo = 0, hi = nb;
-    while (hi - lo > 1) {
-        uint32_t mid = (lo + hi) >> 1;
-        if (offs[mid] <= pos) lo = mid; else hi = mid;
-    }
-    return lo;
+__device__ __forceinline__ uint32_t accum_first_bucket(const uint32_t* __restrict__ seg_bucket, uint32_t lane, uint32_t nb) {
+    const uint32_t b = seg_bucket[lane];
+    return b < nb ? b : nb - 1;
 }
 
 typedef __attribute__((address_space(3))) char* lds_char_ptr;
@@ -131,7 +127,7 @@
 #endif
 __global__ void __launch_bounds__(kAccumBlock, KZG_ACCUM_MIN_BLOCKS)
 k_bucket_accumulate(const uint4* __restrict__ table, const uint32_t* __restrict__ sorted, const uint32_t* __restrict__ offs,
-                    uint32_t nb, uint32_t lanes, uint4* __restrict__ buckets, uint4* __restrict__ part_a,
+                    const uint32_t* __restrict__ seg_bucket, uint32_t nb, uint32_t lanes, uint4* __restrict__ buckets, uint4* __restrict__ part_a,
                     uint4* __restrict__ part_b, unsigned long long* __restrict__ clk) {
     asm volatile("" ::: "v175");
     const bool stamp = clk != nullptr && (threadIdx.x & 63) == 0;
@@ -144,15 +140,15 @@
     const uint32_t start = (uint32_t)start64;
     const uint32_t end = (M - start < L) ? M : start + L;
 
-    uint32_t b = bucket_of(offs, nb, start);
-    uint32_t b_beg = offs[b], b_end = offs[b + 1];
-    uint32_t b_end_next = offs[(b + 2 <= nb) ? b + 2 : nb];
     uint32_t run_start = start;
     XYZZ30 acc = xyzz30_inf();
     const uint32_t wave_slot = accum_wave_slot();
     uint32_t ref = accum_ref(sorted, start);
     uint32_t ref_next = accum_ref(sorted, min(start + 1, M - 1));
     accum_issue_gather(table, wave_slot, ref);
+    uint32_t b = accum_first_bucket(seg_bucket, lane, nb);
+    uint32_t b_beg = offs[b], b_end = offs[b + 1];
+    uint32_t b_end_next = offs[(b + 2 <= nb) ? b + 2 : nb];
     for (uint32_t e = start; e < end; e++) {
         const bool wave_flushed = __builtin_amdgcn_ballot_w64(e == b_end) != 0;
         if (e == b_end) {
@@ -234,7 +230,8 @@
 
 __global__ void __launch_bounds__(kAccumBlock, 2) k_bucket_accumulate_pairs(const uint4* __restrict__ table,
                                                                             const uint32_t* __restrict__ sorted,
-                                                                            const uint32_t* __restrict__ offs, uint32_t nb,
+                                                                            const uint32_t* __restrict__ offs,
+                                                                            const uint32_t* __restrict__ seg_bucket, uint32_t nb,
                                                                             uint32_t lanes, uint4* __restrict__ buckets,
                                                                             uint4* __restrict__ part_a,
                                                                             uint4* __restrict__ part_b,
@@ -270,14 +267,15 @@
         return r;
     };
 
-    uint32_t b = bucket_of(offs, nb, start);
-    uint32_t b_end = offs[b + 1];
+    uint32_t b, b_end;
     Fq run = fq_one();
     {
         uint32_t r0 = sorted[start], r1 = start + 1 < end ? sorted[start + 1] : 0u;
         uint32_t r0n = start + 2 < end ? sorted[start + 2] : 0u, r1n = start + 3 < end ? sorted[start + 3] : 0u;
         dma(slot0, r0, 0, 4);
         dma(slot1, r1, 0, 4);
+        b = accum_first_bucket(seg_bucket, lane, nb);
+        b_end = offs[b + 1];
         for (uint32_t j = 0; j < J; j++) {
             const uint32_t e0 = start + 2 * j, e1 = e0 + 1;
             while (b_end <= e0) {
@@ -322,9 +320,11 @@
     Fq inv = run;
     fq_inv_call(&inv);
 
-    b = bucket_of(offs, nb, end - 1);
+    while (b_end <= end - 1) {
+        b++;
+        b_end = offs[b + 1];
+    }
     uint32_t b_beg = offs[b];
-    b_end = offs[b + 1];
     XYZZ30 acc = xyzz30_inf();
     auto flush = [&]() {
         uint4* dst;
@@ -467,13 +467,13 @@
 }
 
 void launch_bucket_accumulate(hipStream_t s, const void* d_table, const uint32_t* d_sorted, const uint32_t* d_offs,
-                              uint32_t nb, uint32_t lanes, void* d_buckets, void* d_part_a, void* d_part_b,
+                              const uint32_t* d_seg_bucket, uint32_t nb, uint32_t lanes, void* d_buckets, void* d_part_a, void* d_part_b,
                               uint32_t lds_reserve_bytes, void* d_pair_scratch, uint64_t max_refs, void* d_clock) {
     if (!lanes) return;
     if (accumulate_pairs_enabled() && d_pair_scratch && max_refs / lanes >= 16) {
         hipLaunchKernelGGL(k_bucket_accumulate_pairs, dim3(lanes / kAccumBlock), dim3(kAccumBlock),
                            (kAccumBlock / 64) * 16 * 64 * 16 , s,
-                           reinterpret_cast<const uint4*>(d_table), d_sorted, d_offs, nb, lanes,
+                           reinterpret_cast<const uint4*>(d_table), d_sorted, d_offs, d_seg_bucket, nb, lanes,
                            reinterpret_cast<uint4*>(d_buckets), reinterpret_cast<uint4*>(d_part_a),
                            reinterpret_cast<uint4*>(d_part_b), reinterpret_cast<uint4*>(d_pair_scratch));
         return;
@@ -482,7 +482,7 @@
     lds_reserve_bytes = lds_reserve_bytes / (256 / kAccumBlock);
     if (lds_reserve_bytes < need) lds_reserve_bytes = need;
     hipLaunchKernelGGL(k_bucket_accumulate, dim3(lanes / kAccumBlock), dim3(kAccumBlock), lds_reserve_bytes, s,
-                       reinterpret_cast<const uint4*>(d_table), d_sorted, d_offs, nb, lanes,
+                       reinterpret_cast<const uint4*>(d_table), d_sorted, d_offs, d_seg_bucket, nb, lanes,
                        reinterpret_cast<uint4*>(d_buckets), reinterpret_cast<uint4*>(d_part_a),
                        reinterpret_cast<uint4*>(d_part_b), reinterpret_cast<unsigned long long*>(d_clock));
 }
diff --git a/kzg_poly_commit_exploration_amd/csrc/msm_sort.hip b/kzg_poly_commit_exploration_amd/csrc/msm_sort.hip
--- a/kzg_poly_commit_exploration_amd/csrc/msm_sort.hip
+++ b/kzg_poly_commit_exploration_amd/csrc/msm_sort.hip
@@ -215,12 +215,14 @@
 constexpr uint32_t kWsPrefix = kMaxCoarse + 8;
 constexpr uint32_t kWsBinFill = 2 * kMaxCoarse + 32;
 constexpr uint32_t kWsTable = 3 * kMaxCoarse + 64;
-uint32_t sort_workspace_words() { return kWsTable + kFineMaxChunks * (uint32_t)kFineMax + 64; }
+constexpr uint32_t kWsSegBucket = kWsTable + kFineMaxChunks * (uint32_t)kFineMax + 64;
+uint32_t sort_workspace_words() { return kWsSegBucket + kMaxAccumLanes; }
+uint32_t sort_seg_bucket_offset() { return kWsSegBucket; }
 uint32_t sort_workspace_zero_words() { return kWsTable; }
 
 template <int BLOCK>
 KZG_DEV void spread_tile_cursors(uint32_t coarse_bins, const uint32_t* __restrict__ d_cnt, const uint32_t* __restrict__ d_binfill,
-                                 uint32_t ch, uint32_t* __restrict__ d_binstart, uint32_t* __restrict__ d_prefix,
+                                 uint32_t ch, uint32_t fine_cap, uint32_t* __restrict__ d_binstart, uint32_t* __restrict__ d_prefix,
                                  uint32_t* __restrict__ d_total, u32* s_cur , u32* s_scan ) {
     const uint32_t t = threadIdx.x;
     constexpr uint32_t kStripes = kMaxCoarse / BLOCK;
@@ -241,7 +243,7 @@
         __syncthreads();
         if (q < coarse_bins) s_cur[q] = start + below[s];
         if (blockIdx.x == 0) {
-            const u32 nch = q < coarse_bins ? (all[s] + ch - 1) / ch : 0u;
+            const u32 nch = q < coarse_bins && all[s] > fine_cap ? (all[s] + ch - 1) / ch : 0u;
             u32 chunk_total;
             const u32 cstart = chunk_carry + block_exclusive_scan_n<BLOCK>(nch, s_scan, chunk_total);
             __syncthreads();
@@ -266,12 +268,12 @@
                                                             uint32_t tile, uint32_t tiles, uint32_t fine_bits,
                                                             uint32_t coarse_bins, const uint32_t* __restrict__ d_cnt ,
                                                             const uint32_t* __restrict__ d_binfill ,
-                                                            uint32_t ch, uint32_t* __restrict__ d_binstart,
+                                                            uint32_t ch, uint32_t fine_cap, uint32_t* __restrict__ d_binstart,
                                                             uint32_t* __restrict__ d_prefix, uint32_t* __restrict__ d_total,
                                                             uint64_t* __restrict__ d_pairs, int packed) {
     __shared__ u32 s_cur[kMaxCoarse];
     __shared__ u32 s_scan[kRecodeBlock];
-    spread_tile_cursors<kRecodeBlock>(coarse_bins, d_cnt, d_binfill, ch, d_binstart, d_prefix, d_total, s_cur, s_scan);
+    spread_tile_cursors<kRecodeBlock>(coarse_bins, d_cnt, d_binfill, ch, fine_cap, d_binstart, d_prefix, d_total, s_cur, s_scan);
     const uint64_t base = (uint64_t)blockIdx.x * tile;
     const uint64_t total = (uint64_t)bg.n * bg.batch;
     const u32 fine_mask = (1u << fine_bits) - 1u;
@@ -323,7 +325,7 @@
                                                                   BatchGeom bg, uint32_t table_stride, MsmConfig cfg,
                                                                   uint32_t tile, uint32_t fine_bits, uint32_t coarse_bins,
                                                                   const uint32_t* __restrict__ d_cnt, const uint32_t* __restrict__ d_binfill,
-                                                                  uint32_t ch, uint32_t* __restrict__ d_binstart,
+                                                                  uint32_t ch, uint32_t fine_cap, uint32_t* __restrict__ d_binstart,
                                                                   uint32_t* __restrict__ d_prefix, uint32_t* __restrict__ d_total,
                                                                   uint32_t* __restrict__ d_pairs32) {
     __shared__ u32 s_cur[kMaxCoarse];
@@ -332,7 +334,7 @@
     __shared__ u32 s_scan[kStageBlock];
     __shared__ u32 s_stage[kStageSlots];
     __shared__ uint16_t s_sbin[kStageSlots];
-    spread_tile_cursors<kStageBlock>(coarse_bins, d_cnt, d_binfill, ch, d_binstart, d_prefix, d_total, s_cur, s_scan);
+    spread_tile_cursors<kStageBlock>(coarse_bins, d_cnt, d_binfill, ch, fine_cap, d_binstart, d_prefix, d_total, s_cur, s_scan);
     const uint32_t t = threadIdx.x;
     const uint64_t base = (uint64_t)blockIdx.x * tile;
     const uint64_t total = (uint64_t)bg.n * bg.batch;
@@ -458,6 +460,23 @@
     if (threadIdx.x < fine) d_table[(size_t)c.base * fine + (size_t)threadIdx.x * c.nch + c.j] = s_hist[threadIdx.x];
 }
 
+template <int BLOCK>
+KZG_DEV void fill_seg_buckets(const u32* s_start, uint32_t nkeys, uint32_t bucket0, uint32_t rs, uint32_t re, uint32_t M,
+                              uint32_t lanes, uint32_t* __restrict__ d_seg) {
+    const uint32_t L = accumulate_seg_len(M, lanes);
+    const uint32_t l1 = (re + L - 1) / L;
+#pragma unroll 1
+    for (uint32_t l = (rs + L - 1) / L + threadIdx.x; l < l1; l += BLOCK) {
+        const uint32_t pos = l * L - rs;
+        uint32_t lo = 0, hi = nkeys;
+        while (hi - lo > 1) {
+            const uint32_t mid = (lo + hi) >> 1;
+            if (s_start[mid] <= pos) lo = mid; else hi = mid;
+        }
+        d_seg[l] = bucket0 + lo;
+    }
+}
+
 __global__ void __launch_bounds__(kSortBlock) k_fine_binscan(const uint32_t* __restrict__ d_binstart, uint32_t fine_bits,
                                                              const uint32_t* __restrict__ d_prefix,
                                                              uint32_t* __restrict__ d_table, uint32_t* __restrict__ d_offs) {
@@ -467,7 +486,7 @@
     const uint32_t base = d_prefix[bin], nch = d_prefix[bin + 1] - base;
     const uint32_t rs = d_binstart[bin];
     if (nch == 0) {
-        if (t < fine) d_offs[bin * fine + t] = rs;
+        if (d_binstart[bin + 1] == rs && t < fine) d_offs[bin * fine + t] = rs;
         return;
     }
     if (nch <= kFineLocal) return;
@@ -494,7 +513,8 @@
                                                              const uint32_t* __restrict__ d_prefix,
                                                              const uint32_t* __restrict__ d_table,
                                                              uint32_t* __restrict__ d_offs,
-                                                             uint32_t* __restrict__ d_sorted) {
+                                                             uint32_t* __restrict__ d_sorted, uint32_t lanes,
+                                                             uint32_t* __restrict__ d_seg) {
     __shared__ u32 s_cur[kFineMax];
     __shared__ u32 s_cnt[kFineMax];
     __shared__ u32 s_ref[kFineStage];
@@ -504,7 +524,7 @@
     const uint32_t fine = 1u << fine_bits;
     const uint32_t t = threadIdx.x;
     {
-        u32 mine = 0;
+        u32 mine = 0, first = 0;
         if (c.nch <= kFineLocal) {
             u32 row = 0, front = 0;
             if (t < fine) {
@@ -519,12 +539,21 @@
             const u32 key_start = d_binstart[c.bin] + block_exclusive_scan_256(row, s_ref, total);
             __syncthreads();
             mine = key_start + front;
+            first = key_start;
             if (c.j == 0 && t < fine) d_offs[c.bin * fine + t] = key_start;
         } else if (t < fine) {
             mine = d_table[(size_t)c.base * fine + (size_t)t * c.nch + c.j];
+            first = mine;
             if (c.j == 0) d_offs[c.bin * fine + t] = mine;
         }
         if (t < fine) s_cur[t] = mine;
+        if (c.j == 0) {
+            const uint32_t rs = d_binstart[c.bin];
+            if (t < fine) s_cnt[t] = first - rs;
+            __syncthreads();
+            fill_seg_buckets<kSortBlock>(s_cnt, fine, c.bin * fine, rs, d_binstart[c.bin + 1], d_binstart[coarse_bins], lanes, d_seg);
+            __syncthreads();
+        }
     }
     for (uint32_t r0 = c.beg; r0 < c.end; r0 += kFineStage) {
         const uint32_t r1 = (c.end - r0 < kFineStage) ? c.end : r0 + kFineStage;
@@ -590,6 +619,98 @@
     }
 }
 
+constexpr int kFineBinBlock = 256;
+constexpr uint32_t kFineBinRegs = 124;
+constexpr uint32_t kFineBinStage = 16384;
+constexpr uint32_t kFineBinGroup = 8;
+static_assert(kFineBinBlock == kFineMax, "one lane per fine key in the scan");
+typedef u32 FineBinQuad __attribute__((ext_vector_type(4)));
+struct __attribute__((packed, aligned(4))) FineBinQuadOut { u32 w[4]; };
+static uint32_t fine_bin_pairs(bool packed) {
+    static const bool on = [] { const char* v = std::getenv("KZG_FINE_BIN"); return !(v && v[0] == '0'); }();
+    return on ? (uint32_t)kFineBinBlock * (kFineBinRegs / (packed ? 1u : 2u)) : 0u;
+}
+
+template <bool kPacked>
+__global__ void __launch_bounds__(kFineBinBlock) k_fine_bin(const typename SortPair<kPacked>::type* __restrict__ d_pairs,
+                                                            const uint32_t* __restrict__ d_binstart, uint32_t fine_bits,
+                                                            uint32_t coarse_bins, uint32_t fine_cap, uint32_t lanes,
+                                                            uint32_t* __restrict__ d_offs, uint32_t* __restrict__ d_sorted,
+                                                            uint32_t* __restrict__ d_seg) {
+    constexpr uint32_t kSlots = kFineBinRegs / (kPacked ? 1u : 2u);
+    __shared__ u32 s_start[kFineMax];
+    __shared__ u32 s_cur[kFineMax];
+    __shared__ u32 s_scan[kFineBinBlock];
+    __shared__ __attribute__((aligned(16))) u32 s_stage[kFineBinStage];
+    const uint32_t bin = blockIdx.x, t = threadIdx.x;
+    const uint32_t rs = d_binstart[bin], cnt = d_binstart[bin + 1] - rs;
+    if (cnt == 0 || cnt > fine_cap) return;
+    const uint32_t fine = 1u << fine_bits;
+    s_cur[t] = 0;
+    __syncthreads();
+    uint32_t mine = cnt > t ? (cnt - t + kFineBinBlock - 1) / kFineBinBlock : 0u;
+    typename SortPair<kPacked>::type pr[kSlots];
+#pragma unroll
+    for (uint32_t q = 0; q < kSlots; q++) {
+        const uint32_t e = q * kFineBinBlock + t;
+        pr[q] = d_pairs[rs + (e < cnt ? e : cnt - 1)];
+    }
+    asm volatile("" : "+v"(mine));
+#pragma unroll
+    for (uint32_t q = 0; q < kSlots; q++)
+        if (q < mine) atomicAdd(&s_cur[SortPair<kPacked>::key(pr[q])], 1u);
+    __syncthreads();
+    u32 total;
+    const u32 first = block_exclusive_scan_256(s_cur[t], s_scan, total);
+    s_start[t] = first;
+    s_cur[t] = first;
+    if (t < fine) d_offs[bin * fine + t] = rs + first;
+    __syncthreads();
+    fill_seg_buckets<kFineBinBlock>(s_start, fine, bin * fine, rs, rs + cnt, d_binstart[coarse_bins], lanes, d_seg);
+    u32 placed[(kSlots + 31) / 32];
+#pragma unroll
+    for (uint32_t w = 0; w < (kSlots + 31) / 32; w++) placed[w] = mine >= 32 * w + 32 ? 0u : (mine <= 32 * w ? ~0u : ~0u << (mine - 32 * w));
+    for (uint32_t lo = 0; lo < cnt; lo += kFineBinStage) {
+        const uint32_t hi = cnt - lo < kFineBinStage ? cnt : lo + kFineBinStage;
+        const uint32_t kmax = (uint32_t)__syncthreads_count(s_start[t] < hi);
+#pragma unroll
+        for (uint32_t q0 = 0; q0 < kSlots; q0 += kFineBinGroup) {
+            u32 pos[kFineBinGroup];
+#pragma unroll
+            for (uint32_t j = 0; j < kFineBinGroup; j++) {
+                const uint32_t q = q0 + j;
+                pos[j] = ~0u;
+                if (q < kSlots && !((placed[q / 32] >> (q % 32)) & 1u)) {
+                    asm volatile("" : "+v"(pr[q]));
+                    const u32 key = SortPair<kPacked>::key(pr[q]);
+                    if (key < kmax) pos[j] = atomicAdd(&s_cur[key], 1u);
+                }
+            }
+#pragma unroll
+            for (uint32_t j = 0; j < kFineBinGroup; j++) {
+                const uint32_t q = q0 + j;
+                if (q < kSlots && pos[j] < hi) {
+                    s_stage[pos[j] - lo] = SortPair<kPacked>::ref(pr[q]);
+                    placed[q / 32] |= 1u << (q % 32);
+                }
+            }
+        }
+        __syncthreads();
+        if (t < kmax && s_cur[t] > hi) s_cur[t] = hi;
+        u32* const out = d_sorted + rs + lo;
+        const uint32_t m = hi - lo, m4 = m & ~3u;
+#pragma unroll 2
+        for (uint32_t i = 4 * t; i < m4; i += 4 * kFineBinBlock) {
+            const FineBinQuad v = *reinterpret_cast<const FineBinQuad*>(&s_stage[i]);
+            FineBinQuadOut o;
+            o.w[0] = v.x; o.w[1] = v.y; o.w[2] = v.z; o.w[3] = v.w;
+            *reinterpret_cast<FineBinQuadOut*>(out + i) = o;
+        }
+        if (m4 + t < m) out[m4 + t] = s_stage[m4 + t];
+        __syncthreads();
+    }
+}
+
 template <int N>
 __device__ __forceinline__ u32 block_exclusive_scan_n(u32 v, u32* lds, u32& total) {
     int t = threadIdx.x;
@@ -614,7 +735,8 @@
                                                                 uint32_t table_stride, MsmConfig cfg,
                                                                 uint32_t* __restrict__ d_offs,
                                                                 uint32_t* __restrict__ d_sorted,
-                                                                uint32_t* __restrict__ d_header) {
+                                                                uint32_t* __restrict__ d_header, uint32_t lanes,
+                                                                uint32_t* __restrict__ d_seg) {
     __shared__ u32 s_hist[kSmallSortBuckets];
     if (blockIdx.x == 0 && threadIdx.x < kHeavyHeaderBytes / 4) d_header[threadIdx.x] = 0;
     __shared__ u32 s_part[kSmallSortBlock];
@@ -654,6 +776,8 @@
     }
     if (t == kSmallSortBlock - 1) d_offs[nb] = s_part[t];
     __syncthreads();
+    if (blockIdx.x == 0) fill_seg_buckets<kSmallSortBlock>(s_hist, nb, 0u, 0u, s_part[kSmallSortBlock - 1], s_part[kSmallSortBlock - 1], lanes, d_seg);
+    __syncthreads();
     const uint32_t b_lo = (uint32_t)((uint64_t)nb * blockIdx.x / gridDim.x), b_hi = (uint32_t)((uint64_t)nb * (blockIdx.x + 1) / gridDim.x);
     for (uint32_t i = t; i < n; i += kSmallSortBlock) {
         u32 k[8];
@@ -669,14 +793,15 @@
 
 bool launch_bucket_sort(hipStream_t s, const uint32_t* d_scalars, int is_mont, uint32_t n, uint32_t batch,
                         uint64_t stride, uint32_t table_stride, MsmConfig cfg, uint32_t* d_cnt, uint32_t* d_ws,
-                        uint64_t* d_pairs, uint32_t* d_offs, uint32_t* d_sorted, uint32_t* d_header) {
+                        uint64_t* d_pairs, uint32_t* d_offs, uint32_t* d_sorted, uint32_t* d_header, uint32_t lanes) {
     if (n == 0 || batch == 0) return false;
+    uint32_t* d_seg = d_ws + kWsSegBucket;
     static const bool small_path = [] { const char* v = std::getenv("KZG_SMALL_SORT"); return !(v && v[0] == '0'); }();
     if (small_path && batch == 1 && n <= kSmallSortScalars && cfg.nb <= kSmallSortBuckets) {
         uint32_t groups = n / 256;
         groups = groups < 1 ? 1 : (groups > 8 ? 8 : groups);
         hipLaunchKernelGGL(k_sort_small, dim3(groups), dim3(kSmallSortBlock), 0, s, d_scalars, is_mont, n, table_stride, cfg, d_offs,
-                           d_sorted, d_header);
+                           d_sorted, d_header, lanes, d_seg);
         return true;
     }
     const uint32_t nb_total = cfg.nb * batch;
@@ -690,17 +815,24 @@
     const uint32_t ch = fine_chunk_len(max_pairs);
     const uint32_t max_chunks = (uint32_t)((max_pairs + ch - 1) / ch) + g.coarse_bins;
     uint32_t* d_binfill = d_ws + kWsBinFill;
+    const uint32_t fine_cap = fine_bin_pairs(g.packed);
     hipLaunchKernelGGL(k_sort_count, dim3(g.tiles), dim3(kRecodeBlock), 0, s, d_scalars, is_mont, bg, cfg, g.tile,
                        g.fine_bits, g.coarse_bins, d_cnt, d_binfill, d_header);
     static const bool staged = [] { const char* v = std::getenv("KZG_SPREAD_STAGED"); return !(v && v[0] == '0'); }();
     if (g.packed && staged && cfg.max_digits <= kStageSlots)
         hipLaunchKernelGGL(k_sort_spread_staged, dim3(g.tiles), dim3(kStageBlock), 0, s, d_scalars, is_mont, bg, table_stride, cfg,
-                           g.tile, g.fine_bits, g.coarse_bins, d_cnt, d_binfill, ch, d_binstart, d_prefix, d_total,
+                           g.tile, g.fine_bits, g.coarse_bins, d_cnt, d_binfill, ch, fine_cap, d_binstart, d_prefix, d_total,
                            reinterpret_cast<uint32_t*>(d_pairs));
     else
         hipLaunchKernelGGL(k_sort_spread, dim3(g.tiles), dim3(kRecodeBlock), 0, s, d_scalars, is_mont, bg, table_stride, cfg,
-                           g.tile, g.tiles, g.fine_bits, g.coarse_bins, d_cnt, d_binfill, ch, d_binstart, d_prefix, d_total, d_pairs,
+                           g.tile, g.tiles, g.fine_bits, g.coarse_bins, d_cnt, d_binfill, ch, fine_cap, d_binstart, d_prefix, d_total, d_pairs,
                            g.packed ? 1 : 0);
+    if (fine_cap && g.packed)
+        hipLaunchKernelGGL(k_fine_bin<true>, dim3(g.coarse_bins), dim3(kFineBinBlock), 0, s, reinterpret_cast<const uint32_t*>(d_pairs),
+                           d_binstart, g.fine_bits, g.coarse_bins, fine_cap, lanes, d_offs, d_sorted, d_seg);
+    else if (fine_cap)
+        hipLaunchKernelGGL(k_fine_bin<false>, dim3(g.coarse_bins), dim3(kFineBinBlock), 0, s, d_pairs, d_binstart, g.fine_bits,
+                           g.coarse_bins, fine_cap, lanes, d_offs, d_sorted, d_seg);
     if (g.packed)
         hipLaunchKernelGGL(k_fine_count<true>, dim3(max_chunks), dim3(kSortBlock), 0, s, reinterpret_cast<const uint32_t*>(d_pairs),
                            d_binstart, g.fine_bits, g.coarse_bins, ch, d_prefix, d_table, d_binfill);
@@ -710,10 +842,10 @@
     hipLaunchKernelGGL(k_fine_binscan, dim3(g.coarse_bins), dim3(kSortBlock), 0, s, d_binstart, g.fine_bits, d_prefix, d_table, d_offs);
     if (g.packed)
         hipLaunchKernelGGL(k_fine_scatter<true>, dim3(max_chunks), dim3(kSortBlock), 0, s, reinterpret_cast<const uint32_t*>(d_pairs),
-                           d_binstart, g.fine_bits, g.coarse_bins, ch, d_prefix, d_table, d_offs, d_sorted);
+                           d_binstart, g.fine_bits, g.coarse_bins, ch, d_prefix, d_table, d_offs, d_sorted, lanes, d_seg);
     else
         hipLaunchKernelGGL(k_fine_scatter<false>, dim3(max_chunks), dim3(kSortBlock), 0, s, d_pairs, d_binstart, g.fine_bits,
-                           g.coarse_bins, ch, d_prefix, d_table, d_offs, d_sorted);
+                           g.coarse_bins, ch, d_prefix, d_table, d_offs, d_sorted, lanes, d_seg);
     return true;
 }
 
```
